# warwick-hpsc/MG-CFD-app-plain

Hardware: AMD Instinct MI355X
Metric: Medges/s (compute_flux_edge) + MG V-cycle wall-s (higher is better)
Workload: dtype f64; 1 GPU; M6-L0-like synthetic level (67^3 jittered lattice, permuted ids): 300763 nodes / 888822 internal edges per GPU, flux + update sweep, no MG; numerics=exact (bit-identical to the reference), parallelism=1 GPU, workload_kind=level0

## Files before the change

include/mgcfd.h:

```cpp
#ifndef MGCFD_H
#define MGCFD_H

#include <stdint.h>

#ifdef __cplusplus
extern "C" {
#endif

#define MGCFD_NVAR 5
#define MGCFD_RK 3

#define MGCFD_MESH_FVCORR 0
#define MGCFD_MESH_M6_WING 2
#define MGCFD_MESH_LA_CASCADE 3
#define MGCFD_MESH_ROTOR_37 4

#define MGCFD_OK 0
#define MGCFD_ERR_ARG 1
#define MGCFD_ERR_IO 2
#define MGCFD_ERR_HIP 3
#define MGCFD_ERR_NAN 4
#define MGCFD_ERR_NEG_DENSITY 5
#define MGCFD_ERR_NEG_ENERGY 6
#define MGCFD_ERR_VALIDATION 7

enum { MGCFD_LOOP_FLUX = 0, MGCFD_LOOP_UPDATE, MGCFD_LOOP_COMPUTE_STEP, MGCFD_LOOP_TIME_STEP,
       MGCFD_LOOP_RESTRICT, MGCFD_LOOP_PROLONG, MGCFD_LOOP_INDIRECT_RW, MGCFD_NUM_LOOPS };

enum { MGCFD_ARR_VARIABLES = 0, MGCFD_ARR_OLD_VARIABLES, MGCFD_ARR_FLUXES, MGCFD_ARR_RESIDUALS,
       MGCFD_ARR_STEP_FACTORS, MGCFD_ARR_VOLUMES,
       MGCFD_ARR_STAGE  };

enum {
    MGCFD_OPT_EXACT = 0,
    MGCFD_OPT_TIMING = 1,
    MGCFD_OPT_INDIRECT_RW = 2,
    MGCFD_OPT_CHECK_INVALID = 3,
    MGCFD_OPT_FLUX_VARIANT = 4,
    MGCFD_OPT_FUSE_UPDATE = 5,
    MGCFD_OPT_GRAPH = 6,
    MGCFD_OPT_RANK_SPLIT = 7,
    MGCFD_OPT_STAGE_WG4 = 8
};

typedef struct { int64_t a, b; double x, y, z; } mgcfd_edge;

typedef struct {
    int64_t nel;
    int64_t n_edges;
    int64_t n_internal, n_boundary, n_wall;
    int64_t internal_start, boundary_start, wall_start;
    const double *volumes;
    const double *coords;
    const mgcfd_edge *edges;
    const int64_t *mg_map;
    int64_t mgc;
} mgcfd_level_desc;

typedef struct mgcfd_mesh mgcfd_mesh;
typedef struct mgcfd_solver mgcfd_solver;

const char *mgcfd_last_error(void);
int mgcfd_abi_version(void);
int mgcfd_device_warm_up(int device);

int mgcfd_mesh_load(const char *input_dat, const char *directory, int duplicate, mgcfd_mesh **out);
#define MGCFD_MESH_LEGACY_ORDERING 1
int mgcfd_mesh_load_ex(const char *input_dat, const char *directory, int duplicate, int flags, mgcfd_mesh **out);
void mgcfd_mesh_free(mgcfd_mesh *m);
int mgcfd_mesh_num_levels(const mgcfd_mesh *m);
int mgcfd_mesh_variant(const mgcfd_mesh *m);
int mgcfd_mesh_size(const mgcfd_mesh *m);
int mgcfd_mesh_level(const mgcfd_mesh *m, int level, mgcfd_level_desc *out);

int mgcfd_write_array(const char *path, const double *data, int64_t nel, int ncols);
int mgcfd_identify_differences(const double *test_values, const double *master_values, int64_t nel,
                               int mesh_variant, int64_t *first_bad);

int mgcfd_create(const mgcfd_level_desc *levels, int nlevels, int mesh_variant, int device,
                 mgcfd_solver **out);
int mgcfd_create_from_mesh(const mgcfd_mesh *m, int device, mgcfd_solver **out);
int mgcfd_create_partitioned(const mgcfd_level_desc *levels, int nlevels, int mesh_variant, int device,
                             const int64_t *n_owned, mgcfd_solver **out);
int mgcfd_create_partitioned_mg(const mgcfd_level_desc *levels, int nlevels, int mesh_variant, int device,
                                const int64_t *n_owned, const int64_t *const *order_keys, mgcfd_solver **out);
int mgcfd_plan_audit(const mgcfd_level_desc *levels, int nlevels, int mesh_variant, const int64_t *n_owned,
                     const int64_t *const *order_keys, char *report, int64_t report_cap);
void mgcfd_destroy(mgcfd_solver *s);
int mgcfd_set_option(mgcfd_solver *s, int option, int value);
int mgcfd_level_has_edge_once(const mgcfd_solver *s, int level, int *yes);
int mgcfd_level_has_half_rows(const mgcfd_solver *s, int level, int *yes);
int mgcfd_level_has_order_free(const mgcfd_solver *s, int level, int *yes);
int mgcfd_level_stage_wg4(const mgcfd_solver *s, int level, int *yes);
int mgcfd_level_tiling(const mgcfd_solver *s, int level, int64_t out[10]);
int mgcfd_get_option(const mgcfd_solver *s, int option, int *value);
int mgcfd_set_stream(mgcfd_solver *s, void *hip_stream);
int mgcfd_synchronize(mgcfd_solver *s);
int mgcfd_num_levels(const mgcfd_solver *s);
int64_t mgcfd_level_nel(const mgcfd_solver *s, int level);
int64_t mgcfd_level_num_internal_edges(const mgcfd_solver *s, int level);
int mgcfd_get_far_field(const mgcfd_solver *s, double *out17);

int mgcfd_copy_old_variables(mgcfd_solver *s, int level);
int mgcfd_compute_step_factor(mgcfd_solver *s, int level);
int mgcfd_compute_flux_edge(mgcfd_solver *s, int level);
int mgcfd_compute_boundary_flux_edge(mgcfd_solver *s, int level);
int mgcfd_compute_wall_flux_edge(mgcfd_solver *s, int level);
int mgcfd_compute_fluxes(mgcfd_solver *s, int level);
int mgcfd_time_step(mgcfd_solver *s, int level, int j);
int mgcfd_zero_fluxes(mgcfd_solver *s, int level);
int mgcfd_indirect_rw(mgcfd_solver *s, int level);
int mgcfd_residual(mgcfd_solver *s, int level);
int mgcfd_calc_rms(mgcfd_solver *s, int level, double *rms);
int mgcfd_check_for_invalid_variables(mgcfd_solver *s, int level, int64_t *bad_cell);
int mgcfd_pending_invalid_state(mgcfd_solver *s, int64_t *bad_cell);
int mgcfd_restrict(mgcfd_solver *s, int fine_level);
int mgcfd_prolong(mgcfd_solver *s, int fine_level);

int mgcfd_smooth(mgcfd_solver *s, int level, int sweeps);
int mgcfd_run_cycles(mgcfd_solver *s, int cycles, double *rms_out);
int mgcfd_invalid_state_location(const mgcfd_solver *s, int64_t *cell, int *cycle);

int mgcfd_get_array(mgcfd_solver *s, int level, int which, double *out);
int mgcfd_set_array(mgcfd_solver *s, int level, int which, const double *in);
int mgcfd_array_devptr(mgcfd_solver *s, int level, int which, void **devptr, int64_t *count);
int mgcfd_array_written(mgcfd_solver *s, int level, int which);
int mgcfd_get_edges(mgcfd_solver *s, int level, mgcfd_edge *out);
int mgcfd_accept_restricted(mgcfd_solver *s, int fine_level, const void *dev_src);

int mgcfd_get_loop_iters(const mgcfd_solver *s, int level, int64_t out[MGCFD_NUM_LOOPS]);
int mgcfd_get_loop_times(mgcfd_solver *s, int level, double out_seconds[MGCFD_NUM_LOOPS]);
int mgcfd_reset_monitoring(mgcfd_solver *s);
int mgcfd_get_flux_kernel_time(mgcfd_solver *s, int level, double *avg_seconds, int64_t *launches);

int mgcfd_bench_flux(mgcfd_solver *s, int level, int launches, double *avg_seconds);
int mgcfd_bench_indirect_rw(mgcfd_solver *s, int level, int launches, double *avg_seconds);
int mgcfd_bench_stream_ceiling(mgcfd_solver *s, int level, int launches, double *avg_seconds);

int mgcfd_step_factor_local(mgcfd_solver *s, int level);
int mgcfd_step_factor_min_devptr(mgcfd_solver *s, int level, void **devptr);
int mgcfd_step_factor_apply(mgcfd_solver *s, int level);
int mgcfd_sweep_begin(mgcfd_solver *s, int level);
int mgcfd_step_factor_partials_devptr(mgcfd_solver *s, int level, void **devptr, int *count);
int mgcfd_sweep_stage(mgcfd_solver *s, int level, int j, int partials);
int mgcfd_sweep_begin_partials(mgcfd_solver *s, int level);
int mgcfd_sweep_end_partials(mgcfd_solver *s, int level);
int mgcfd_sweep_flux0(mgcfd_solver *s, int level);
int mgcfd_sweep_end(mgcfd_solver *s, int level);
int mgcfd_halo_plan(mgcfd_solver *s, int level, int64_t n, const int64_t *node_ids, int *plan);
int mgcfd_halo_pack(mgcfd_solver *s, int level, int plan, int which, void *dev_buf);
int mgcfd_halo_unpack(mgcfd_solver *s, int level, int plan, int which, const void *dev_buf);
int mgcfd_residual_sumsq(mgcfd_solver *s, int level, void **devptr);

typedef struct mgcfd_group mgcfd_group;
int mgcfd_rccl_unique_id(void *out128);
int mgcfd_rank_attach_rccl(mgcfd_solver *s, int rank, int world, const void *id128);
int mgcfd_rank_detach(mgcfd_solver *s);
int mgcfd_rank_set_halo(mgcfd_solver *s, int level, int n_peers, const int *peers, const int64_t *send_counts,
                        const int64_t *const *send_ids, const int64_t *recv_counts, const int64_t *const *recv_ids);
int mgcfd_rank_halo_info(const mgcfd_solver *s, int level, int64_t out[4]);
int mgcfd_rank_info(const mgcfd_solver *s, int out[4]);
int mgcfd_rank_graph_status(const mgcfd_solver *s, int level, int64_t out[3]);
int mgcfd_rank_exchange(mgcfd_solver *s, int level);
int mgcfd_rank_sweeps(mgcfd_solver *s, int level, int sweeps);
int mgcfd_rank_residual_sumsq(mgcfd_solver *s, int level, double *sum_all_ranks);
int mgcfd_rank_attach_plain(mgcfd_solver *s, int rank, int world);
int mgcfd_rank_ipc_export_size(mgcfd_solver *s, int level, int64_t *bytes);
int mgcfd_rank_ipc_export(mgcfd_solver *s, int level, void *out);
int mgcfd_rank_ipc_attach(mgcfd_solver *s, int level, int n_exports, const void *const *exports);
int mgcfd_rank_ipc_status(mgcfd_solver *s, int level, int *timed_out);
int mgcfd_rank_ipc_detach(mgcfd_solver *s, int level);
int mgcfd_group_create(int n, mgcfd_solver *const *solvers, mgcfd_group **out);
void mgcfd_group_destroy(mgcfd_group *g);
int mgcfd_group_exchange(mgcfd_group *g, int level);
int mgcfd_group_sweeps(mgcfd_group *g, int level, int sweeps);
int mgcfd_group_sweeps_rms(mgcfd_group *g, int level, int sweeps, double *rms_of_each);
// ... 10 lines not shown
```

mg-cfd-app-plain_amd/csrc/device_plan.hpp:

```cpp
#pragma once

#include <hip/hip_runtime.h>
#include <cstdint>

#include "preprocess.hpp"

namespace mgcfd {

constexpr int kNumStateFields = 5;
static_assert(sizeof(EdgeW) == 32, "EdgeW must be 32 bytes");
static_assert(sizeof(ProlongW) == 24, "ProlongW must be 24 bytes");

constexpr int kVariantStageWg4 = 1 << 7;

struct FarField {
    double var[5];
    double fc_mx[3], fc_my[3], fc_mz[3], fc_de[3];
};

constexpr int kMaxPushPeers = 8;
struct PushPeers {
    double *base[kMaxPushPeers] = {nullptr, nullptr, nullptr, nullptr, nullptr, nullptr, nullptr, nullptr};
    int64_t stride[kMaxPushPeers] = {0, 0, 0, 0, 0, 0, 0, 0};
    int64_t first[kMaxPushPeers + 1] = {0, 0, 0, 0, 0, 0, 0, 0, 0};
    int n = 0;
};

struct PushFlags {
    unsigned long long *flag[kMaxPushPeers] = {nullptr, nullptr, nullptr, nullptr, nullptr, nullptr, nullptr, nullptr};
    unsigned long long value = 0;
    int n = 0;
};
struct StagePush {
    const int32_t *send_ptr = nullptr;
    const int8_t *send_peer = nullptr;
    const int32_t *send_target = nullptr;
    PushPeers peers;
    PushFlags flags;
    unsigned *ticket = nullptr;
    int32_t n_boundary = 0;
};

constexpr int kMaxIpcRanks = 16;
struct FlagRows { int row[kMaxIpcRanks] = {0, 0, 0, 0, 0, 0, 0, 0, 0, 0, 0, 0, 0, 0, 0, 0}; int n = 0; };
struct MinPublish {
    double *mins[kMaxIpcRanks] = {nullptr, nullptr, nullptr, nullptr, nullptr, nullptr, nullptr, nullptr, nullptr, nullptr, nullptr, nullptr, nullptr, nullptr, nullptr, nullptr};
    unsigned long long *flag[kMaxIpcRanks] = {nullptr, nullptr, nullptr, nullptr, nullptr, nullptr, nullptr, nullptr, nullptr, nullptr, nullptr, nullptr, nullptr, nullptr, nullptr, nullptr};
    int world = 0, me = 0, parity = 0;
    unsigned long long value = 0;
};

struct FusedStep {
    double rk_div = 1.0;
    double *step_factors = nullptr;
    const double *old_variables = nullptr;
    double *q_out = nullptr;
    const double *partial_min = nullptr;
    int n_partial = 0;
    const double *volumes = nullptr;
    double *residuals = nullptr;
    const int32_t *old_of_new = nullptr;
    unsigned long long *err = nullptr;
    int check = 0;
    const double *vin_flux = nullptr;
    double vin_div = 4.0;
    int check_vin = 0;
    double *sumsq_partial = nullptr;
    double *next_partial_min = nullptr;
    const double *cbrt_vol = nullptr;
    double *next_legacy_sf = nullptr;
    const int32_t *tile_list = nullptr;
    int32_t n_list = 0;
    int64_t nel_active = 0;
};

struct SumTask {
    const double *partial = nullptr;
    int n = 0;
    double *out = nullptr;
    double *ring = nullptr;
    int *count = nullptr;
    int cap = 0;
};

struct TailPlan {
    const int32_t *rows_main = nullptr;
    const int32_t *tile_ptr = nullptr;
    const double2 *rec = nullptr;
    const int32_t *begin = nullptr, *count = nullptr;
    double2 *flux = nullptr;
};

struct DevicePlan {
    int64_t nel = 0;
    int64_t stride = 0;
    int32_t n_slices = 0;
    int32_t *slice_row0 = nullptr, *rows_int = nullptr, *rows_bnd = nullptr, *nbr = nullptr;
    double *w = nullptr;
    int32_t n_tiles = 0;
    int32_t pad_row = 0;
    int32_t pad_chunk = 0;
    uint16_t *nbr16 = nullptr;
    int32_t *tile_halo = nullptr;
    int32_t *tile_ovf_ptr = nullptr, *tile_ovf = nullptr;
    int vin_ok = 0;
    int lds_complete = 0;
    int32_t halo_max = 0;
    int edge_once = 0;
    int32_t *te_chunk_ptr = nullptr, *te_count = nullptr;
    uint16_t *te_slots = nullptr, *gat16 = nullptr;
    double *te_w = nullptr;
    double *te_w3 = nullptr;
    int half = 0;
    int free_rows = 0;
    int32_t hr_max_rows = 0;
    int free_wide = 0;
    int32_t *free_halo = nullptr;
    int32_t hr_pad_row = 0;
    int32_t *hr_row0 = nullptr;
    uint32_t *hr_code = nullptr;
    uint16_t *hg16 = nullptr;
    double *hr_w = nullptr;
    int has_tail = 0;
    TailPlan tail;
    int64_t n_edges = 0, n_edges_pad = 0;
    int32_t *fe_ab = nullptr, *row_edge = nullptr;
    double *fe_w = nullptr, *edge_flux = nullptr;
    int32_t *old_of_new = nullptr;
    int32_t *child_ptr = nullptr, *child = nullptr;
    int32_t *child4 = nullptr;
    double *pro_w = nullptr;
    int32_t *pro_p = nullptr;
    int pro_tiled = 0;
    int32_t *pro_tile_n = nullptr, *pro_tile_ids = nullptr;
    uint16_t *pro_s16 = nullptr, *pro_own16 = nullptr;
    int32_t *pro_parent = nullptr;
    double *pro_wsum = nullptr;
};

inline bool stage_wg4_fits(const DevicePlan &p) { return !p.has_tail && p.halo_max <= kTileCap4 - kTile; }

}
```

mg-cfd-app-plain_amd/csrc/kernels.hip:

```cpp
#include <hip/hip_runtime.h>
#include <algorithm>
#include <cstdlib>
#include <stdexcept>
#include <stdint.h>
#include <type_traits>

#include "device_plan.hpp"

#ifndef MGCFD_KERNEL_NS
#error "compile with -DMGCFD_KERNEL_NS=exact|fast"
#endif

namespace mgcfd {
namespace MGCFD_KERNEL_NS {

#ifdef MGCFD_PHASES
__device__ unsigned long long g_phase[4096 * 8];
__device__ unsigned long long g_phase_abs[4096 * 8];
#define PH_MARK(k) do { if (threadIdx.x == 0) { unsigned long long now_ = wall_clock64(); g_phase[(blockIdx.x & 4095) * 8 + (k)] += now_ - ph_last_; ph_last_ = now_; g_phase_abs[(blockIdx.x & 4095) * 8 + 1 + (k)] = now_; } } while (0)
#define PH_BEGIN() unsigned long long ph_last_ = wall_clock64(); if (threadIdx.x == 0) { g_phase[(blockIdx.x & 4095) * 8 + 7] += 1ull; g_phase_abs[(blockIdx.x & 4095) * 8] = ph_last_; \
        g_phase_abs[(blockIdx.x & 4095) * 8 + 7] = (static_cast<unsigned long long>(__builtin_amdgcn_s_getreg(20 | (0 << 6) | (31 << 11))) << 32) | __builtin_amdgcn_s_getreg(4 | (0 << 6) | (31 << 11)); }
#else
#define PH_MARK(k) do { } while (0)
#define PH_BEGIN() do { } while (0)
// ... 432 lines not shown
            sf_next = 0.5 * dt;
        } else if (fs.next_legacy_sf) {
            const Derived d = derive(rho, mx, my, mz, en);
            fs.next_legacy_sf[i] = 0.5 / (sqrt(fs.volumes[i]) * (d.speed + d.c));
        }
    }
    if (fs.next_partial_min || fs.sumsq_partial) {
        __shared__ double s_next[2][kBlock / 64];
        sf_next = wave_min(sf_next);
        ss = wave_sum(ss);
        if ((threadIdx.x & 63) == 0) { s_next[0][threadIdx.x >> 6] = sf_next; s_next[1][threadIdx.x >> 6] = ss; }
        __syncthreads();
        if (threadIdx.x == 0) {
            double m = s_next[0][0], sum = s_next[1][0];
            for (int wv = 1; wv < kBlock / 64; wv++) { m = fmin(m, s_next[0][wv]); sum += s_next[1][wv]; }
            if (fs.next_partial_min) fs.next_partial_min[t] = m;
            if (fs.sumsq_partial) fs.sumsq_partial[t] = sum;
        }
    }
}

__device__ __forceinline__ void boundary_rows(const NodeQ &me, const FluxC &fm, const FarField &ff,
                                              const uint16_t *__restrict__ nbr16, const double *__restrict__ w,
                                              int64_t first_row, int32_t n_bnd, int lane, int classes, double &a0,
                                              double &a1, double &a2, double &a3, double &a4)
{
    for (int32_t r = 0; r < n_bnd; r++) {
        const EdgeRow e = load_row<false>(nbr16, w, first_row + r, lane);
        const double fx = e.fx, fy = e.fy, fz = e.fz;
        if (e.code == kT16Wall && (classes & 2)) {
            a0 += 0.0;
            a1 += fx * me.p;
            a2 += fy * me.p;
            a3 += fz * me.p;
            a4 += 0.0;
        } else if (e.code == kT16Far && (classes & 4)) {
            a0 += fx * (ff.var[1] + me.mx) + fy * (ff.var[2] + me.my) + fz * (ff.var[3] + me.mz);
            a4 += fx * (ff.fc_de[0] + fm.ex) + fy * (ff.fc_de[1] + fm.ey) + fz * (ff.fc_de[2] + fm.ez);
            a1 += fx * (ff.fc_mx[0] + fm.xx) + fy * (ff.fc_mx[1] + fm.xy) + fz * (ff.fc_mx[2] + fm.xz);
            a2 += fx * (ff.fc_my[0] + fm.xy) + fy * (ff.fc_my[1] + fm.yy) + fz * (ff.fc_my[2] + fm.yz);
            a3 += fx * (ff.fc_mz[0] + fm.xz) + fy * (ff.fc_mz[1] + fm.yz) + fz * (ff.fc_mz[2] + fm.zz);
        }
    }
}

struct FluxTileLds {
    double2 tile[kTileCap * kLdsRecD2];
    double s_pm[kBlock / 64];
    double s_next[2][kBlock / 64];
};
struct FluxTileLds4 {
    double2 tile[kTileCap4 * kLdsRec80D2];
    double s_pm[kBlock / 64];
    double s_next[2][kBlock / 64];
};
static_assert(sizeof(FluxTileLds4) <= 160 * 1024 / 4, "four workgroups per CU");
static_assert(kTileCap4 - kTile < kBlock, "one halo id per thread");

template <int WMODE, bool FUSE, bool ACC, int ROLE, bool TAIL, bool PUSH, bool SLIM = false, typename Lds = FluxTileLds>
__device__ __forceinline__ void
flux_tile_body(Lds &lds, const unsigned block,
               const double *__restrict__ q, const int32_t *__restrict__ tile_halo, uint32_t n_tiles, int32_t pad_row,
               int64_t stride, int64_t nel, const int32_t *__restrict__ slice_row0,
               const int32_t *__restrict__ rows_int, const int32_t *__restrict__ rows_bnd,
               const uint16_t *__restrict__ nbr16, const double *__restrict__ w,
               const int32_t *__restrict__ tile_ovf_ptr, const int32_t *__restrict__ tile_ovf, const FarField &ff,
               double *__restrict__ fluxes, int classes, const FusedStep &fs, const TailPlan &tp,
               const uint16_t *__restrict__ gat16, const int32_t *__restrict__ te_chunk_ptr, const double *__restrict__ te_w3,
               const StagePush &push ,
               const bool block_is_tile = false )
{
    constexpr bool LOADK = WMODE == 1;
    static_assert(!PUSH || FUSE, "only a fused stage sends its message");
    PH_BEGIN();
    constexpr bool IDXW = WMODE == 2;
    static_assert(!(IDXW && TAIL), "indexed weights: levels without long rows only");
    static_assert(!SLIM || (!TAIL && !IDXW && !PUSH && ROLE != 5), "80-byte records: the stages without long rows, indexed weights, message or absorbed stage");
    double2 *const tile = lds.tile;

    double min_dt = 0.0;
    constexpr int kPartPre = 6;
    double *const s_pm = lds.s_pm;
    double pmv[kPartPre];

    const int tid = threadIdx.x;
    const int lane = tid & 63;
    unsigned t = block_is_tile ? block : xcd_contiguous_block(block, n_tiles);
    if (PUSH) {
        const unsigned nb = unsigned(push.n_boundary);
        t = block < nb ? block : nb + xcd_contiguous_block(block - nb, n_tiles - nb);
    }
    if (FUSE && fs.tile_list) t = unsigned(fs.tile_list[t]);
    const int64_t base = int64_t(t) * kTile;
    const int64_t i = base + tid;
    const int32_t slice = __builtin_amdgcn_readfirstlane(static_cast<int32_t>(i >> 6));

    const int32_t *hrow = tile_halo + int64_t(t) * kHaloStride;
    const int32_t hid = hrow[tid];
    const int32_t hid2 = (!SLIM && ROLE != 5 && tid < kHaloStride - kBlock) ? hrow[kBlock + tid] : -1;
    const int32_t row0 = slice_row0[slice];
    const int32_t n_int = (classes & 1) ? (TAIL ? tp.rows_main : rows_int)[slice] : 0;
    const int32_t n_bnd = rows_bnd[slice];
    const bool has_halo = hid >= 0;
    const int64_t hnode = has_halo ? int64_t(hid) : i;
    double o0, o1, o2, o3, o4, g0, g1, g2, g3, g4;
    EdgeRow e0, e1;
    RowRef i0{}, i1{}, i2{}, i3{};
    const double *tw = nullptr;
    if (IDXW) {
        i0 = load_ref(nbr16, gat16, n_int > 0 ? row0 : pad_row, lane);
        i1 = load_ref(nbr16, gat16, n_int > 1 ? row0 + 1 : pad_row, lane);
        i2 = load_ref(nbr16, gat16, n_int > 2 ? row0 + 2 : pad_row, lane);
        i3 = load_ref(nbr16, gat16, n_int > 3 ? row0 + 3 : pad_row, lane);
        tw = te_w3 + int64_t(te_chunk_ptr[t]) * (kEdgeChunk * 3);
    }
    if (FUSE && ROLE == 5) {
#pragma unroll
        for (int u = 0; u < kPartPre; u++) {
            const int k = threadIdx.x + u * kBlock;
            pmv[u] = fs.partial_min[k < fs.n_partial ? k : fs.n_partial - 1];
        }
        const double *od = fs.old_variables, *fl = fs.vin_flux;
        const double b0 = od[i], b1 = od[stride + i], b2 = od[2 * stride + i], b3 = od[3 * stride + i], b4 = od[4 * stride + i];
        const double f0 = fl[i], f1 = fl[stride + i], f2 = fl[2 * stride + i], f3 = fl[3 * stride + i], f4 = fl[4 * stride + i];
        const double vo = fs.volumes[i];
        const double c0 = od[hnode], c1 = od[stride + hnode], c2 = od[2 * stride + hnode], c3 = od[3 * stride + hnode],
                     c4 = od[4 * stride + hnode];
        const double h0 = fl[hnode], h1 = fl[stride + hnode], h2 = fl[2 * stride + hnode], h3 = fl[3 * stride + hnode],
                     h4 = fl[4 * stride + hnode];
        const double vh = fs.volumes[hnode];
        if (IDXW) { e0 = gather_weights(tw, i0); e1 = gather_weights(tw, i1); }
        else {
            e0 = load_row<LOADK>(nbr16, w, n_int > 0 ? row0 : pad_row, lane);
            e1 = load_row<LOADK>(nbr16, w, n_int > 1 ? row0 + 1 : pad_row, lane);
        }
        double pm = pmv[0];
#pragma unroll
        for (int u = 1; u < kPartPre; u++) pm = fmin(pm, pmv[u]);
        for (int k = threadIdx.x + kPartPre * kBlock; k < fs.n_partial; k += kBlock) pm = fmin(pm, fs.partial_min[k]);
        pm = wave_min(pm);
        if (lane == 0) s_pm[tid >> 6] = pm;
        __syncthreads();
        min_dt = s_pm[0];
        for (int wv = 1; wv < kBlock / 64; wv++) min_dt = fmin(min_dt, s_pm[wv]);
        const double fo = (min_dt / vo) / fs.vin_div, fh = (min_dt / vh) / fs.vin_div;
        o0 = b0 + fo * f0; o1 = b1 + fo * f1; o2 = b2 + fo * f2; o3 = b3 + fo * f3; o4 = b4 + fo * f4;
        g0 = c0 + fh * h0; g1 = c1 + fh * h1; g2 = c2 + fh * h2; g3 = c3 + fh * h3; g4 = c4 + fh * h4;
        if (fs.check_vin && i < nel) {
            const bool finite = isfinite(o0) && isfinite(o1) && isfinite(o2) && isfinite(o3) && isfinite(o4);
            int code = 0;
            if (!finite) code = 1;
            else if (o0 < 0.0) code = 2;
            else if (o4 < 0.0) code = 3;
            if (code) atomicMin(fs.err, err_key(fs.check_vin, fs.old_of_new[i], code));
        }
    } else {
        o0 = q[i]; o1 = q[stride + i]; o2 = q[2 * stride + i]; o3 = q[3 * stride + i]; o4 = q[4 * stride + i];
        g0 = q[hnode]; g1 = q[stride + hnode]; g2 = q[2 * stride + hnode]; g3 = q[3 * stride + hnode]; g4 = q[4 * stride + hnode];
        if (IDXW) { e0 = gather_weights(tw, i0); e1 = gather_weights(tw, i1); }
        else {
            e0 = load_row<LOADK>(nbr16, w, n_int > 0 ? row0 : pad_row, lane);
            if (!SLIM) e1 = load_row<LOADK>(nbr16, w, n_int > 1 ? row0 + 1 : pad_row, lane);
        }
    }
    if (FUSE && ROLE == 0) {
#pragma unroll
        for (int u = 0; u < kPartPre; u++) {
            const int k = threadIdx.x + u * kBlock;
            pmv[u] = fs.partial_min[k < fs.n_partial ? k : fs.n_partial - 1];
        }
    }
    const NodeQ me = make_nodeq(o0, o1, o2, o3, o4);
    lds_put_rec<SLIM>(tile, uint32_t(tid), me);
    const uint32_t hslot = (SLIM && tid >= kTileCap4 - kTile) ? uint32_t(tid) : uint32_t(kTile + tid);
    lds_put_rec<SLIM>(tile, hslot, make_nodeq(g0, g1, g2, g3, g4));
    if (hid2 >= 0) lds_store_record(tile, uint32_t(kTile + kBlock + tid), load_and_derive(q, stride, hid2));

    const FluxC fm_pre = flux_contribution(me);
    double a0 = 0.0, a1 = 0.0, a2 = 0.0, a3 = 0.0, a4 = 0.0;
    if (ACC) {
        a0 = fluxes[i]; a1 = fluxes[stride + i]; a2 = fluxes[2 * stride + i];
        a3 = fluxes[3 * stride + i]; a4 = fluxes[4 * stride + i];
    }
    const int32_t ovf0 = tile_ovf_ptr[t];
    if (FUSE && ROLE == 0) {
        double pm = pmv[0];
#pragma unroll
        for (int u = 1; u < kPartPre; u++) pm = fmin(pm, pmv[u]);
        for (int k = threadIdx.x + kPartPre * kBlock; k < fs.n_partial; k += kBlock) pm = fmin(pm, fs.partial_min[k]);
        pm = wave_min(pm);
        if (lane == 0) s_pm[tid >> 6] = pm;
    }
    PH_MARK(0);
    __syncthreads();
    PH_MARK(1);

#define MGCFD_ROW_PAIR()                                                                                     \
    do {                                                                                                     \
            const uint32_t s0 = e0.code & kT16SlotMask, s1 = e1.code & kT16SlotMask;                         \
            const bool v0 = s0 != kT16Pad, v1 = s1 != kT16Pad;                                               \
            const bool o0 = v0 && s0 >= uint32_t(kTileCap), o1 = v1 && s1 >= uint32_t(kTileCap);             \
            NodeQ n0, n1;                                                                                    \
            if (!TAIL && __builtin_expect(__any(o0 || o1), 0)) {       \
                n0 = o0 ? load_and_derive(q, stride, tile_ovf[ovf0 + int32_t(s0) - kTileCap])                \
                        : lds_load_record(tile, v0 ? s0 : uint32_t(tid));                                    \
                n1 = o1 ? load_and_derive(q, stride, tile_ovf[ovf0 + int32_t(s1) - kTileCap])                \
                        : lds_load_record(tile, v1 ? s1 : uint32_t(tid));                                    \
            } else {                                                                                         \
                n0 = lds_load_record(tile, v0 ? s0 : uint32_t(tid));                                         \
                n1 = lds_load_record(tile, v1 ? s1 : uint32_t(tid));                                         \
            }                                                                                                \
            Flux5 f0, f1;                                                                                    \
            f0 = edge_flux<LOADK>(me, fm_pre, n0, e0);                                                       \
            f1 = edge_flux<LOADK>(me, fm_pre, n1, e1);                                                       \
            if (ACC || TAIL) {                                                                               \
                a0 = v0 ? a0 + f0.d : a0;   a1 = v0 ? a1 + f0.mx : a1;   a2 = v0 ? a2 + f0.my : a2;          \
                a3 = v0 ? a3 + f0.mz : a3;  a4 = v0 ? a4 + f0.en : a4;                                       \
                a0 = v1 ? a0 + f1.d : a0;   a1 = v1 ? a1 + f1.mx : a1;   a2 = v1 ? a2 + f1.my : a2;          \
                a3 = v1 ? a3 + f1.mz : a3;  a4 = v1 ? a4 + f1.en : a4;                                       \
            } else {                                                                                         \
                a0 += f0.d; a1 += f0.mx; a2 += f0.my; a3 += f0.mz; a4 += f0.en;                              \
                a0 += f1.d; a1 += f1.mx; a2 += f1.my; a3 += f1.mz; a4 += f1.en;                              \
            }                                                                                                \
    } while (0)
    int32_t tl_b = 0, tl_e = 0, tl_nb = 0, tl_nc = 0;
    double2 tl_r0 = make_double2(0.0, 0.0), tl_r1 = tl_r0, tl_r2 = tl_r0;
    if (TAIL && (classes & 1)) {
        tl_b = tp.tile_ptr[t]; tl_e = tp.tile_ptr[t + 1];
        tl_nb = tp.begin[i]; tl_nc = tp.count[i];
        const int32_t e_first = tl_b + tid;
        if (e_first < tl_e) { tl_r0 = tp.rec[3 * int64_t(e_first)]; tl_r1 = tp.rec[3 * int64_t(e_first) + 1]; tl_r2 = tp.rec[3 * int64_t(e_first) + 2]; }
    }
    double r0 = 0.0, r1 = 0.0, r2 = 0.0, r3 = 0.0, r4 = 0.0, sfv = 0.0;
#define MGCFD_ROW_ONE()                                                                                      \
    do {                                                                                                     \
            const uint32_t s0 = e0.code & kT16SlotMask;                                                      \
            const bool v0 = s0 != kT16Pad;                                                                   \
            const NodeQ n0 = lds_get_record80(tile, v0 ? s0 : uint32_t(tid));                              \
            const Flux5 f0 = edge_flux<LOADK>(me, fm_pre, n0, e0);                                           \
            if (ACC) {                                                                                       \
                a0 = v0 ? a0 + f0.d : a0;   a1 = v0 ? a1 + f0.mx : a1;   a2 = v0 ? a2 + f0.my : a2;          \
                a3 = v0 ? a3 + f0.mz : a3;  a4 = v0 ? a4 + f0.en : a4;                                       \
            } else {                                                                                         \
                a0 += f0.d; a1 += f0.mx; a2 += f0.my; a3 += f0.mz; a4 += f0.en;                              \
            }                                                                                                \
    } while (0)
    if (SLIM) {
        int32_t r = 0;
        for (; r + 1 < n_int; r++) {
            const EdgeRow e1n = load_row<LOADK>(nbr16, w, row0 + r + 1, lane);
            MGCFD_ROW_ONE();
            e0 = e1n;
        }
        if (FUSE) {
            if (ROLE == 0) {
                r0 = me.rho; r1 = me.mx; r2 = me.my; r3 = me.mz; r4 = me.en;
            } else {
                r0 = fs.old_variables[i]; r1 = fs.old_variables[stride + i]; r2 = fs.old_variables[2 * stride + i];
                r3 = fs.old_variables[3 * stride + i]; r4 = fs.old_variables[4 * stride + i];
            }
            sfv = (ROLE == 0 ? fs.volumes : fs.step_factors)[i];
        }
        if (r < n_int) MGCFD_ROW_ONE();
    } else
    {
        int32_t r = 0;
        if (IDXW) {
            for (; r + 2 < n_int; r += 2) {
                const RowRef i4 = load_ref(nbr16, gat16, r + 4 < n_int ? row0 + r + 4 : pad_row, lane);
                const RowRef i5 = load_ref(nbr16, gat16, r + 5 < n_int ? row0 + r + 5 : pad_row, lane);
                const EdgeRow e2 = gather_weights(tw, i2), e3 = gather_weights(tw, i3);
                MGCFD_ROW_PAIR();
                e0 = e2; e1 = e3; i2 = i4; i3 = i5;
            }
        } else
        for (; r + 2 < n_int; r += 2) {
            const EdgeRow e2 = load_row<LOADK>(nbr16, w, row0 + r + 2, lane);
            const EdgeRow e3 = load_row<LOADK>(nbr16, w, r + 3 < n_int ? row0 + r + 3 : pad_row, lane);
            MGCFD_ROW_PAIR();
            e0 = e2; e1 = e3;
        }
        if (FUSE) {
            if (ROLE == 0) {
                r0 = me.rho; r1 = me.mx; r2 = me.my; r3 = me.mz; r4 = me.en;
            } else {
                r0 = fs.old_variables[i]; r1 = fs.old_variables[stride + i]; r2 = fs.old_variables[2 * stride + i];
                r3 = fs.old_variables[3 * stride + i]; r4 = fs.old_variables[4 * stride + i];
            }
            sfv = ((ROLE == 0 || ROLE == 5) ? fs.volumes : fs.step_factors)[i];
        }
        if (r < n_int) MGCFD_ROW_PAIR();
    }
#undef MGCFD_ROW_PAIR
#undef MGCFD_ROW_ONE
    PH_MARK(2);

    if (TAIL && (classes & 1) && tl_e > tl_b) {
        const int32_t last0 = tl_b + ((tl_e - tl_b - 1) / kBlock) * kBlock;
        int32_t e = tl_b + tid;
        double2 r0 = tl_r0, r1 = tl_r1, r2 = tl_r2;
        Flux5 fl;
        fl.d = 0.0; fl.mx = 0.0; fl.my = 0.0; fl.mz = 0.0; fl.en = 0.0;
        while (e < tl_e) {
            const double2 c0 = r0, c1 = r1, c2 = r2;
            const int32_t en = e + kBlock;
            if (en < tl_e) { r0 = tp.rec[3 * int64_t(en)]; r1 = tp.rec[3 * int64_t(en) + 1]; r2 = tp.rec[3 * int64_t(en) + 2]; }
            const uint32_t word = static_cast<uint32_t>(__double_as_longlong(c2.x));
            const uint32_t own = word & 0xFFFFu;
            if (own != kT16Pad) {
                EdgeRow er;
                er.code = word >> 16;
                er.fx = c0.x; er.fy = c0.y; er.fz = c1.x; er.k = LOADK ? c1.y : 0.0;
                const uint32_t s = er.code & kT16SlotMask;
                const NodeQ mo = lds_load_record(tile, own);
                const NodeQ ot = s >= uint32_t(kTileCap) ? load_and_derive(q, stride, tile_ovf[ovf0 + int32_t(s) - kTileCap])
                                                         : lds_load_record(tile, s);
                const Flux5 f = edge_flux<LOADK>(mo, flux_contribution(mo), ot, er);
                if (e >= last0) {
                    fl = f;
                } else {
                    double2 *out = tp.flux + 3 * int64_t(e);
                    out[0] = make_double2(f.d, f.mx); out[1] = make_double2(f.my, f.mz); out[2] = make_double2(f.en, 0.0);
                }
            }
            e = en;
        }
        asm volatile("s_waitcnt vmcnt(0)" ::: "memory");
        __syncthreads();
        tile[3 * tid] = make_double2(fl.d, fl.mx); tile[3 * tid + 1] = make_double2(fl.my, fl.mz); tile[3 * tid + 2] = make_double2(fl.en, 0.0);
        __syncthreads();
        const int32_t n_glob = min(tl_nc, max(0, last0 - tl_nb));
#define MGCFD_ADD_ENTRIES(in, count)                                                                              \
        do {                                                                                                      \
            int32_t k_ = 0;                                                                                       \
            for (; k_ + 3 <= (count); k_ += 3) {            \
                const double2 u0 = in[0], u1 = in[1], u2 = in[2], v0 = in[3], v1 = in[4], v2 = in[5],              \
                              w0 = in[6], w1 = in[7], w2 = in[8];                                                 \
                in += 9;                                                                                          \
                a0 += u0.x; a1 += u0.y; a2 += u1.x; a3 += u1.y; a4 += u2.x;                                       \
                a0 += v0.x; a1 += v0.y; a2 += v1.x; a3 += v1.y; a4 += v2.x;                                       \
                a0 += w0.x; a1 += w0.y; a2 += w1.x; a3 += w1.y; a4 += w2.x;                                       \
            }                                                                                                     \
            for (; k_ < (count); k_++) {                                                                          \
                const double2 u0 = in[0], u1 = in[1], u2 = in[2];                                                 \
                in += 3;                                                                                          \
                a0 += u0.x; a1 += u0.y; a2 += u1.x; a3 += u1.y; a4 += u2.x;                                       \
            }                                                                                                     \
        } while (0)
        if (n_glob > 0) {
            const double2 *in = tp.flux + 3 * int64_t(tl_nb);
            MGCFD_ADD_ENTRIES(in, n_glob);
        }
        {
            const double2 *in = tile + 3 * (tl_nb + n_glob - last0);
            const int32_t n_lds = tl_nc - n_glob;
            MGCFD_ADD_ENTRIES(in, n_lds);
        }
#undef MGCFD_ADD_ENTRIES
    }

    if ((classes & 6) && n_bnd > 0) {
        const int32_t first_bnd = rows_int[slice];
        const FluxC fm = fm_pre;
        for (int32_t r = 0; r < n_bnd; r++) {
            const EdgeRow e = load_row<false>(nbr16, w, int64_t(row0) + first_bnd + r, lane);
            const double fx = e.fx, fy = e.fy, fz = e.fz;
            if (e.code == kT16Wall && (classes & 2)) {
                a0 += 0.0;
                a1 += fx * me.p;
                a2 += fy * me.p;
                a3 += fz * me.p;
                a4 += 0.0;
            } else if (e.code == kT16Far && (classes & 4)) {
                a0 += fx * (ff.var[1] + me.mx) + fy * (ff.var[2] + me.my) + fz * (ff.var[3] + me.mz);
                a4 += fx * (ff.fc_de[0] + fm.ex) + fy * (ff.fc_de[1] + fm.ey) + fz * (ff.fc_de[2] + fm.ez);
                a1 += fx * (ff.fc_mx[0] + fm.xx) + fy * (ff.fc_mx[1] + fm.xy) + fz * (ff.fc_mx[2] + fm.xz);
                a2 += fx * (ff.fc_my[0] + fm.xy) + fy * (ff.fc_my[1] + fm.yy) + fz * (ff.fc_my[2] + fm.yz);
                a3 += fx * (ff.fc_mz[0] + fm.xz) + fy * (ff.fc_mz[1] + fm.yz) + fz * (ff.fc_mz[2] + fm.zz);
            }
        }
    }

    if (!FUSE) {
        if (i < nel) {
            MGCFD_ST_FLUX(fluxes + i, a0); MGCFD_ST_FLUX(fluxes + stride + i, a1); MGCFD_ST_FLUX(fluxes + 2 * stride + i, a2);
            MGCFD_ST_FLUX(fluxes + 3 * stride + i, a3); MGCFD_ST_FLUX(fluxes + 4 * stride + i, a4);
        }
        PH_MARK(3);
        return;
    }
    double sf_next = __longlong_as_double(0x7FF0000000000000LL);
    double ss = 0.0;
    if (i < nel) {
        double sf = sfv;
        if (ROLE == 0 || ROLE == 5) {
            min_dt = s_pm[0];
            for (int wv = 1; wv < kBlock / 64; wv++) min_dt = fmin(min_dt, s_pm[wv]);
            sf = min_dt / sfv;
            fs.step_factors[i] = sf;
        }
        const double factor = sf / fs.rk_div;
        const double rho = r0 + factor * a0, mx = r1 + factor * a1, my = r2 + factor * a2, mz = r3 + factor * a3,
                     en = r4 + factor * a4;
        store_conserved(fs.q_out, stride, i, rho, mx, my, mz, en);
        if (ROLE >= 2 && ROLE <= 4) {
            const double d0 = rho - r0, d1 = mx - r1, d2 = my - r2, d3 = mz - r3, d4 = en - r4;
            if (fs.residuals) {
                MGCFD_ST_STAGE(fs.residuals + i, d0); MGCFD_ST_STAGE(fs.residuals + stride + i, d1); MGCFD_ST_STAGE(fs.residuals + 2 * stride + i, d2);
                MGCFD_ST_STAGE(fs.residuals + 3 * stride + i, d3); MGCFD_ST_STAGE(fs.residuals + 4 * stride + i, d4);
            }
            if (fs.sumsq_partial) ss = (((d0 * d0 + d1 * d1) + d2 * d2) + d3 * d3) + d4 * d4;
        }
        if (fs.check) {
            const bool finite = isfinite(rho) && isfinite(mx) && isfinite(my) && isfinite(mz) && isfinite(en);
            int code = 0;
            if (!finite) code = 1;
            else if (rho < 0.0) code = 2;
            else if (en < 0.0) code = 3;
            if (code) atomicMin(fs.err, err_key(fs.check, fs.old_of_new[i], code));
        }
        if (ROLE == 3) {
            const Derived d = derive(rho, mx, my, mz, en);
            const double dt = fs.cbrt_vol[i] / (d.speed + d.c);
            sf_next = 0.5 * dt;
        } else if (ROLE == 4) {
            const Derived d = derive(rho, mx, my, mz, en);
            fs.next_legacy_sf[i] = 0.5 / (sqrt(fs.volumes[i]) * (d.speed + d.c));
        }
        if (PUSH && block < unsigned(push.n_boundary)) {
            for (int32_t e = push.send_ptr[i]; e < push.send_ptr[i + 1]; e++) {
                const int k = push.send_peer[e];
                const int64_t g = push.send_target[e];
                double *dst = push.peers.base[0];
                int64_t ps = push.peers.stride[0];
#pragma unroll
                for (int p = 1; p < kMaxPushPeers; p++) if (p == k) { dst = push.peers.base[p]; ps = push.peers.stride[p]; }
                dst[g] = rho; dst[ps + g] = mx; dst[2 * ps + g] = my; dst[3 * ps + g] = mz; dst[4 * ps + g] = en;
            }
        }
    }
    if (PUSH && block < unsigned(push.n_boundary)) {
        asm volatile("s_waitcnt vmcnt(0)" ::: "memory");
        __syncthreads();
        if (threadIdx.x == 0) {
            __threadfence_system();
            const unsigned done = __hip_atomic_fetch_add(push.ticket, 1u, __ATOMIC_ACQ_REL, __HIP_MEMORY_SCOPE_AGENT);
            if (done == unsigned(push.n_boundary) - 1u) {
                __hip_atomic_store(push.ticket, 0u, __ATOMIC_RELAXED, __HIP_MEMORY_SCOPE_AGENT);
                __threadfence_system();
#pragma unroll
                for (int p = 0; p < kMaxPushPeers; p++)
                    if (p < push.flags.n) __hip_atomic_store(push.flags.flag[p], push.flags.value, __ATOMIC_RELEASE, __HIP_MEMORY_SCOPE_SYSTEM);
            }
        }
    }
    if (ROLE == 3 || (ROLE >= 2 && ROLE <= 4 && fs.sumsq_partial)) {
        double (*const s_next)[kBlock / 64] = lds.s_next;
        if (ROLE == 3) sf_next = wave_min(sf_next);
        if (fs.sumsq_partial) ss = wave_sum(ss);
        if ((threadIdx.x & 63) == 0) { s_next[0][threadIdx.x >> 6] = sf_next; s_next[1][threadIdx.x >> 6] = ss; }
        __syncthreads();
        if (threadIdx.x == 0) {
            double m = s_next[0][0], sum = s_next[1][0];
            for (int wv = 1; wv < kBlock / 64; wv++) { m = fmin(m, s_next[0][wv]); sum += s_next[1][wv]; }
            if (ROLE == 3) fs.next_partial_min[t] = m;
            if (fs.sumsq_partial) fs.sumsq_partial[t] = sum;
        }
    }
    PH_MARK(3);
}

template <int MINW, int WMODE, bool FUSE, bool ACC, int ROLE, bool TAIL, bool PUSH = false, bool SLIM = false>
__global__ void __launch_bounds__(kBlock, MINW)
k_flux_tile(
            const double *__restrict__ q, const int32_t *__restrict__ tile_halo, uint32_t n_tiles, int32_t pad_row,
            int64_t stride, int64_t nel, const int32_t *__restrict__ slice_row0,
            const int32_t *__restrict__ rows_int, const int32_t *__restrict__ rows_bnd,
            const uint16_t *__restrict__ nbr16, const double *__restrict__ w,
            const int32_t *__restrict__ tile_ovf_ptr, const int32_t *__restrict__ tile_ovf, FarField ff,
            double *__restrict__ fluxes, int classes, FusedStep fs, TailPlan tp,
            const uint16_t *__restrict__ gat16, const int32_t *__restrict__ te_chunk_ptr, const double *__restrict__ te_w3,
            StagePush push)
{
    __shared__ std::conditional_t<SLIM, FluxTileLds4, FluxTileLds> lds;
    flux_tile_body<WMODE, FUSE, ACC, ROLE, TAIL, PUSH, SLIM>(lds, blockIdx.x, q, tile_halo, n_tiles, pad_row, stride, nel, slice_row0, rows_int, rows_bnd, nbr16, w,
                                                       tile_ovf_ptr, tile_ovf, ff, fluxes, classes, fs, tp, gat16, te_chunk_ptr, te_w3, push);
}

struct TileEdge { uint32_t sa, sb; double fx, fy, fz, k; };
constexpr int kGatherPre = 8;

template <bool LOADK>
__device__ __forceinline__ TileEdge load_tile_edge(const uint16_t *__restrict__ te_slots, const double *__restrict__ te_w,
                                                   int64_t chunk, int tid)
{
    TileEdge e;
    e.sa = te_slots[(chunk * 2) * kEdgeChunk + tid];
    e.sb = te_slots[(chunk * 2 + 1) * kEdgeChunk + tid];
    const double *wr = te_w + chunk * (4 * kEdgeChunk) + tid;
    e.fx = wr[0]; e.fy = wr[kEdgeChunk]; e.fz = wr[2 * kEdgeChunk];
    e.k = LOADK ? wr[3 * kEdgeChunk] : 0.0;
    return e;
}

__device__ __forceinline__ TileEdge no_tile_edge()
{
    TileEdge e;
    e.sa = kT16Pad; e.sb = kT16Pad; e.fx = 0.0; e.fy = 0.0; e.fz = 0.0; e.k = 0.0;
    return e;
}

template <bool LOADK, bool FUSE, bool ACC>
__global__ void __launch_bounds__(kBlock, 3)
k_flux_edge_once(const double *__restrict__ q, const int32_t *__restrict__ tile_halo, uint32_t n_tiles, int32_t pad_row,
                 int64_t stride, int64_t nel, const int32_t *__restrict__ te_chunk_ptr,
                 const int32_t *__restrict__ te_count, int32_t pad_chunk, int classes,
                 const int32_t *__restrict__ slice_row0,
                 const int32_t *__restrict__ rows_int, const int32_t *__restrict__ rows_bnd,
                 const uint16_t *__restrict__ nbr16, const double *__restrict__ w, const uint16_t *__restrict__ gat16,
                 const uint16_t *__restrict__ te_slots, const double *__restrict__ te_w,
                 const int32_t *__restrict__ tile_ovf_ptr, const int32_t *__restrict__ tile_ovf, FarField ff,
                 double *__restrict__ fluxes, FusedStep fs)
{
    __shared__ double2 tile[kTileCap * kLdsRecD2];

    double min_dt = 0.0;
    if (FUSE && fs.partial_min) min_dt = block_min_of_partials(fs.partial_min, fs.n_partial);

    const unsigned t = xcd_contiguous_block(blockIdx.x, n_tiles);
    const int tid = threadIdx.x;
    const int lane = tid & 63;
    const int wave_base = tid & ~63;
    const int64_t base = int64_t(t) * kTile;
    const int64_t i = base + tid;
    const int32_t slice = __builtin_amdgcn_readfirstlane(static_cast<int32_t>(i >> 6));

    const int32_t *hrow = tile_halo + int64_t(t) * kHaloStride;
    const int32_t hid = hrow[tid];
    const int32_t hid2 = tid < kHaloStride - kBlock ? hrow[kBlock + tid] : -1;
    const double o0 = q[i], o1 = q[stride + i], o2 = q[2 * stride + i], o3 = q[3 * stride + i], o4 = q[4 * stride + i];
    const int32_t n_te = te_count[t];
    const int64_t chunk0 = te_chunk_ptr[t];
    TileEdge e_cur = load_tile_edge<LOADK>(te_slots, te_w, wave_base < n_te ? chunk0 : pad_chunk, tid);
    TileEdge e_nxt = load_tile_edge<LOADK>(te_slots, te_w, kEdgeChunk + wave_base < n_te ? chunk0 + 1 : pad_chunk, tid);

    const int32_t row0 = slice_row0[slice];
    const int32_t n_int = rows_int[slice];
    const int32_t n_bnd = rows_bnd[slice];
// ... 1154 lines not shown
            double *d = cr + k * 5;
            d[0] = coarse_residuals[c2]; d[1] = coarse_residuals[sc + c2]; d[2] = coarse_residuals[2 * sc + c2];
            d[3] = coarse_residuals[3 * sc + c2]; d[4] = coarse_residuals[4 * sc + c2];
        }
    }
    __syncthreads();

    const double *od = cr + own_slot * 5;
    const double o0 = od[0], o1 = od[1], o2 = od[2], o3 = od[3], o4 = od[4];
    double r0, r1, r2, r3, r4;
    if (parent < 0) {
        r0 = o0; r1 = o1; r2 = o2; r3 = o3; r4 = o4;
    } else {
        r0 = r1 = r2 = r3 = r4 = 0.0;
#define MGCFD_PRO_PAIR(R)                                                                                      \
        do {                                                                                                   \
            const bool v0 = wa0 != 0.0 || wb0 != 0.0;                                                          \
            const bool v1 = ((R) + 1 < n_int) && (wa1 != 0.0 || wb1 != 0.0);                                   \
            const double *xd0 = cr + (v0 ? sl0 : own_slot) * 5, *xd1 = cr + (v1 ? sl1 : own_slot) * 5;         \
            const double x00 = xd0[0], x01 = xd0[1], x02 = xd0[2], x03 = xd0[3], x04 = xd0[4];                 \
            const double x10 = xd1[0], x11 = xd1[1], x12 = xd1[2], x13 = xd1[3], x14 = xd1[4];                 \
            if (v0) {                                                                                          \
                r0 += wa0 * o0; r1 += wa0 * o1; r2 += wa0 * o2; r3 += wa0 * o3; r4 += wa0 * o4;                \
                r0 += wb0 * x00; r1 += wb0 * x01; r2 += wb0 * x02; r3 += wb0 * x03; r4 += wb0 * x04;           \
            }                                                                                                  \
            if (v1) {                                                                                          \
                r0 += wa1 * o0; r1 += wa1 * o1; r2 += wa1 * o2; r3 += wa1 * o3; r4 += wa1 * o4;                \
                r0 += wb1 * x10; r1 += wb1 * x11; r2 += wb1 * x12; r3 += wb1 * x13; r4 += wb1 * x14;           \
            }                                                                                                  \
        } while (0)
        int32_t r = 0;
        for (; r + 2 < n_int; r += 2, wr += 256, sr += 128) {
            const double wa2 = wr[256], wb2 = wr[320], wa3 = wr[384], wb3 = wr[448];
            const uint32_t sl2 = sr[128], sl3 = sr[192];
            MGCFD_PRO_PAIR(r);
            wa0 = wa2; wb0 = wb2; wa1 = wa3; wb1 = wb3; sl0 = sl2; sl1 = sl3;
        }
        if (r < n_int) MGCFD_PRO_PAIR(r);
#undef MGCFD_PRO_PAIR
    }
    double sf = __longlong_as_double(0x7FF0000000000000LL);
    if (active) {
        const double n0 = q0 + (f0 - r0 / ws);
        const double n1 = q1 + (f1 - r1 / ws);
        const double n2 = q2 + (f2 - r2 / ws);
        const double n3 = q3 + (f3 - r3 / ws);
        const double n4 = q4 + (f4 - r4 / ws);
        store_conserved(fine_q, stride, i, n0, n1, n2, n3, n4);
        if (partial_min) sf = local_step_factor(n0, n1, n2, n3, n4, cbrt_vol[i]);
    }
    if (partial_min) block_min_to(sf, partial_min);
}

static inline unsigned grid_for(int64_t n) { return static_cast<unsigned>((n + kBlock - 1) / kBlock); }

void launch_init_variables(hipStream_t st, int64_t stride, const FarField &ff, double *q)
{ hipLaunchKernelGGL(k_init_variables, dim3(grid_for(stride)), dim3(kBlock), 0, st, stride, ff, q); }

void launch_step_factor_local(hipStream_t st, int64_t nel, int64_t stride, const double *q, const double *cbrt_vol,
                              double *sf, double *partial_min, double *old_variables)
{ hipLaunchKernelGGL(k_step_factor_local, dim3(grid_for(nel)), dim3(kBlock), 0, st, nel, stride, q, cbrt_vol, sf, partial_min, old_variables); }

void launch_min_reduce(hipStream_t st, int64_t nel, const double *partial_min, double *out)
{ hipLaunchKernelGGL(k_min_reduce, dim3(1), dim3(kBlock), 0, st, partial_min, int(grid_for(nel)), out); }

void launch_step_factor_apply(hipStream_t st, int64_t nel, const double *min_dt_scalar,
                              const double *volumes, double *sf)
{ hipLaunchKernelGGL(k_step_factor_apply, dim3(grid_for(nel)), dim3(kBlock), 0, st, nel, min_dt_scalar, volumes, sf); }

void launch_step_factor_legacy(hipStream_t st, int64_t nel, int64_t stride, const double *q, const double *volumes, double *sf,
                               double *old_variables)
{ hipLaunchKernelGGL(k_step_factor_legacy, dim3(grid_for(nel)), dim3(kBlock), 0, st, nel, stride, q, volumes, sf, old_variables); }

void launch_flux(hipStream_t st, const DevicePlan &p, const double *q, const FarField &ff, double *fluxes,
                 int classes, int accumulate, int variant, const FusedStep *fused, const StagePush *push)
{
    const dim3 block(kBlock);
    FusedStep fs{};
    if (fused) fs = *fused;
    const bool part = fused && fs.tile_list;
    const int64_t nel_arg = (fused && fs.nel_active > 0) ? fs.nel_active : p.nel;
    const dim3 grid(part ? fs.n_list : p.n_tiles);
    if (part && fs.n_list <= 0) return;

#define MGCFD_TILE_LAUNCH_T(WMODE, FUSE, ACC, ROLE, TAIL)                                                      \
    hipLaunchKernelGGL((k_flux_tile<((TAIL) && ((ACC) || (ROLE) == 5)) ? 2 : 3, WMODE, FUSE, ACC, ROLE, TAIL>), grid, block, 0, st, q, p.tile_halo,     \
                       uint32_t(grid.x), p.pad_row, p.stride, nel_arg, p.slice_row0, p.rows_int, p.rows_bnd, \
                       p.nbr16, p.w, p.tile_ovf_ptr, p.tile_ovf, ff, fluxes, classes, fs, p.tail, p.gat16,     \
                       p.te_chunk_ptr, p.te_w3, StagePush{})
    const bool tail = p.has_tail && (classes & 1);
    if (push && fused && part && !fs.vin_flux) {
        const int role_p = fs.partial_min ? 0 : (fs.next_partial_min ? 3 : (fs.next_legacy_sf ? 4 : (fs.residuals ? 2 : 1)));
#define MGCFD_PUSH_LAUNCH_T(WMODE, ROLE, TAIL)                                                                  \
    hipLaunchKernelGGL((k_flux_tile<3, WMODE, true, false, ROLE, TAIL, true>), grid, block, 0, st, q, p.tile_halo,     \
                       uint32_t(grid.x), p.pad_row, p.stride, nel_arg, p.slice_row0, p.rows_int, p.rows_bnd, \
                       p.nbr16, p.w, p.tile_ovf_ptr, p.tile_ovf, ff, fluxes, classes, fs, p.tail, p.gat16,     \
                       p.te_chunk_ptr, p.te_w3, *push)
#define MGCFD_PUSH_LAUNCH_R(WMODE, TAIL)                                                                        \
    do {                                                                                                       \
        if (role_p == 0) MGCFD_PUSH_LAUNCH_T(WMODE, 0, TAIL);                                                  \
        else if (role_p == 2) MGCFD_PUSH_LAUNCH_T(WMODE, 2, TAIL);                                             \
        else if (role_p == 3) MGCFD_PUSH_LAUNCH_T(WMODE, 3, TAIL);                                             \
        else if (role_p == 4) MGCFD_PUSH_LAUNCH_T(WMODE, 4, TAIL);                                             \
        else MGCFD_PUSH_LAUNCH_T(WMODE, 1, TAIL);                                                              \
    } while (0)
        if (role_p == 0 && q != fs.old_variables) throw std::logic_error("a first stage whose input is not the sweep's start state");
        const bool k_streamed = (variant & 1) == 0;
        if (tail) { if (k_streamed) MGCFD_PUSH_LAUNCH_R(1, true); else MGCFD_PUSH_LAUNCH_R(0, true); }
        else { if (k_streamed) MGCFD_PUSH_LAUNCH_R(1, false); else MGCFD_PUSH_LAUNCH_R(0, false); }
#undef MGCFD_PUSH_LAUNCH_R
#undef MGCFD_PUSH_LAUNCH_T
        return;
    }
    const bool indexed = (variant & 16) && p.edge_once && p.te_w3 && !tail;
#define MGCFD_TILE_LAUNCH_R(LOADK, FUSE, ACC, ROLE)                                                            \
    do {                                                                                                       \
        if (tail) MGCFD_TILE_LAUNCH_T(LOADK ? 1 : 0, FUSE, ACC, ROLE, true);                                   \
        else if (indexed) MGCFD_TILE_LAUNCH_T(2, FUSE, ACC, ROLE, false);                                      \
        else MGCFD_TILE_LAUNCH_T(LOADK ? 1 : 0, FUSE, ACC, ROLE, false);                                       \
    } while (0)
    const int role = !fused ? 1 : (fs.vin_flux ? 5 : fs.partial_min ? 0 : (fs.next_partial_min ? 3 : (fs.next_legacy_sf ? 4 : (fs.residuals ? 2 : 1))));
    if (role == 0 && q != fs.old_variables) throw std::logic_error("a first stage whose input is not the sweep's start state");
#define MGCFD_TILE_LAUNCH(LOADK, FUSE, ACC)                                                                    \
    do {                                                                                                       \
        if (role == 0) MGCFD_TILE_LAUNCH_R(LOADK, FUSE, ACC, 0);                                               \
        else if (role == 2) MGCFD_TILE_LAUNCH_R(LOADK, FUSE, ACC, 2);                                          \
        else if (role == 3) MGCFD_TILE_LAUNCH_R(LOADK, FUSE, ACC, 3);                                          \
        else if (role == 4) MGCFD_TILE_LAUNCH_R(LOADK, FUSE, ACC, 4);                                          \
        else if (role == 5) MGCFD_TILE_LAUNCH_R(LOADK, FUSE, ACC, 5);                                          \
        else MGCFD_TILE_LAUNCH_R(LOADK, FUSE, ACC, 1);                                                         \
    } while (0)
    if ((variant & 4) && !fused && p.edge_flux) {
        if (classes & 1)
            hipLaunchKernelGGL(k_fission_edge_flux, dim3(grid_for(p.n_edges)), block, 0, st, p.n_edges, p.n_edges_pad, p.stride, q,
                               p.fe_ab, p.fe_w, p.edge_flux);
        if (accumulate)
            hipLaunchKernelGGL(k_fission_node_sum<true>, grid, block, 0, st, p.nel, p.stride, p.n_edges_pad, q, p.slice_row0,
                               p.rows_int, p.rows_bnd, p.row_edge, p.nbr16, p.w, p.edge_flux, ff, fluxes, classes);
        else
            hipLaunchKernelGGL(k_fission_node_sum<false>, grid, block, 0, st, p.nel, p.stride, p.n_edges_pad, q, p.slice_row0,
                               p.rows_int, p.rows_bnd, p.row_edge, p.nbr16, p.w, p.edge_flux, ff, fluxes, classes);
        return;
    }
#ifdef MGCFD_ORDER_FREE
    if ((variant & 64) && p.free_rows && (classes & 1) && !(fused && fs.vin_flux) && !part && !(fused && fs.nel_active > 0)) {
#define MGCFD_FREE_LAUNCH_L(FUSE, ACC, CAP, LONG)                                                               \
    hipLaunchKernelGGL((k_flux_free<FUSE, ACC, CAP, LONG>), grid, block, 0, st, q, p.tile_halo, uint32_t(p.n_tiles), \
                       p.hr_pad_row, p.stride, p.nel, p.hr_row0, p.hr_code, p.hr_w, p.slice_row0,               \
                       p.rows_int, p.rows_bnd, p.nbr16, p.w, ff, fluxes, classes, fs)
#define MGCFD_FREE_LAUNCH_C(FUSE, ACC, CAP)                                                                     \
    do { if (p.hr_max_rows > kHalfMaxRows) MGCFD_FREE_LAUNCH_L(FUSE, ACC, CAP, true); else MGCFD_FREE_LAUNCH_L(FUSE, ACC, CAP, false); } while (0)
#define MGCFD_FREE_LAUNCH_W(FUSE, ACC)                                                                          \
    hipLaunchKernelGGL((k_flux_free<FUSE, ACC, kTile + kFreeHaloStride, true, true>), grid, block, 0, st, q, p.free_halo, uint32_t(p.n_tiles), \
                       p.hr_pad_row, p.stride, p.nel, p.hr_row0, p.hr_code, p.hr_w, p.slice_row0,               \
                       p.rows_int, p.rows_bnd, p.nbr16, p.w, ff, fluxes, classes, fs)
        static const bool wg3 = std::getenv("MGCFD_FREE_WG3") && std::atoi(std::getenv("MGCFD_FREE_WG3")) != 0;
#define MGCFD_FREE_LAUNCH(FUSE, ACC)                                                                            \
    do { if (p.free_wide) MGCFD_FREE_LAUNCH_W(FUSE, ACC);                                                       \
         else if (p.halo_max <= kFreeCap4 - kTile && !wg3) MGCFD_FREE_LAUNCH_C(FUSE, ACC, kFreeCap4); else MGCFD_FREE_LAUNCH_C(FUSE, ACC, kTileCap); } while (0)
        const int role_f = !fused ? -1 : (fs.next_legacy_sf ? -1 : (fs.partial_min ? 0 : (fs.next_partial_min ? 3 : ((fs.residuals || fs.sumsq_partial) ? 2 : 1))));
        static const bool no_roles = std::getenv("MGCFD_FREE_NO_ROLES") && std::atoi(std::getenv("MGCFD_FREE_NO_ROLES")) != 0;
        const bool fast_path = !p.free_wide && p.halo_max <= kFreeCap4 - kTile && !wg3 && p.hr_max_rows <= kHalfMaxRows;
#define MGCFD_FREE_LAUNCH_ROLE(ROLE)                                                                            \
    hipLaunchKernelGGL((k_flux_free<true, false, kFreeCap4, false, false, ROLE>), grid, block, 0, st, q, p.tile_halo, uint32_t(p.n_tiles), \
                       p.hr_pad_row, p.stride, p.nel, p.hr_row0, p.hr_code, p.hr_w, p.slice_row0,               \
                       p.rows_int, p.rows_bnd, p.nbr16, p.w, ff, fluxes, classes, fs)
        if (fused && role_f >= 0 && fast_path && !no_roles && !(role_f == 0 && q != fs.old_variables)) {
            if (role_f == 0) MGCFD_FREE_LAUNCH_ROLE(0);
            else if (role_f == 2) MGCFD_FREE_LAUNCH_ROLE(2);
            else if (role_f == 3) MGCFD_FREE_LAUNCH_ROLE(3);
            else MGCFD_FREE_LAUNCH_ROLE(1);
        }
        else if (fused) MGCFD_FREE_LAUNCH(true, false);
        else if (accumulate) MGCFD_FREE_LAUNCH(false, true);
        else MGCFD_FREE_LAUNCH(false, false);
#undef MGCFD_FREE_LAUNCH_ROLE
#undef MGCFD_FREE_LAUNCH_C
#undef MGCFD_FREE_LAUNCH_L
#undef MGCFD_FREE_LAUNCH_W
#undef MGCFD_FREE_LAUNCH
        return;
    }
#endif
    if ((variant & 32) && p.half && (classes & 1) && !(fused && fs.vin_flux) && !part) {
#define MGCFD_HALF_LAUNCH(FUSE, ACC)                                                                            \
    hipLaunchKernelGGL((k_flux_half<FUSE, ACC>), grid, block, 0, st, q, p.tile_halo, uint32_t(p.n_tiles),       \
                       p.hr_pad_row, p.stride, p.nel, p.hr_row0, p.hr_code, p.hr_w, p.hg16, p.slice_row0,       \
                       p.rows_int, p.rows_bnd, p.pad_row, p.nbr16, p.w, ff, fluxes, classes, fs)
        if (fused) MGCFD_HALF_LAUNCH(true, false);
        else if (accumulate) MGCFD_HALF_LAUNCH(false, true);
        else MGCFD_HALF_LAUNCH(false, false);
#undef MGCFD_HALF_LAUNCH
        return;
    }
    const bool loadk = (variant & 1) == 0;
    if ((variant & 2) && p.edge_once && (classes & 1) && !part) {
#define MGCFD_EO_LAUNCH(LOADK, FUSE, ACC)                                                                      \
    hipLaunchKernelGGL((k_flux_edge_once<LOADK, FUSE, ACC>), grid, block, 0, st, q, p.tile_halo,               \
                       uint32_t(p.n_tiles), p.pad_row, p.stride, p.nel, p.te_chunk_ptr, p.te_count,            \
                       p.pad_chunk, classes, p.slice_row0, p.rows_int, p.rows_bnd, p.nbr16, p.w, p.gat16,      \
                       p.te_slots, p.te_w, p.tile_ovf_ptr, p.tile_ovf, ff, fluxes, fs)
        if (fused) {
            if (loadk) MGCFD_EO_LAUNCH(true, true, false); else MGCFD_EO_LAUNCH(false, true, false);
        } else if (accumulate) {
            if (loadk) MGCFD_EO_LAUNCH(true, false, true); else MGCFD_EO_LAUNCH(false, false, true);
        } else {
            if (loadk) MGCFD_EO_LAUNCH(true, false, false); else MGCFD_EO_LAUNCH(false, false, false);
        }
#undef MGCFD_EO_LAUNCH
        return;
    }
#ifndef MGCFD_ORDER_FREE
    if (fused && (variant & kVariantStageWg4) && stage_wg4_fits(p) && !indexed && role != 5) {
#define MGCFD_SLIM_LAUNCH_T(WMODE, ROLE)                                                                        \
    hipLaunchKernelGGL((k_flux_tile<4, WMODE, true, false, ROLE, false, false, true>), grid, block, 0, st, q, p.tile_halo, \
                       uint32_t(grid.x), p.pad_row, p.stride, nel_arg, p.slice_row0, p.rows_int, p.rows_bnd, \
                       p.nbr16, p.w, p.tile_ovf_ptr, p.tile_ovf, ff, fluxes, classes, fs, p.tail, p.gat16,     \
                       p.te_chunk_ptr, p.te_w3, StagePush{})
#define MGCFD_SLIM_LAUNCH_R(WMODE)                                                                              \
    do {                                                                                                       \
        if (role == 0) MGCFD_SLIM_LAUNCH_T(WMODE, 0);                                                          \
        else if (role == 2) MGCFD_SLIM_LAUNCH_T(WMODE, 2);                                                     \
        else if (role == 3) MGCFD_SLIM_LAUNCH_T(WMODE, 3);                                                     \
        else if (role == 4) MGCFD_SLIM_LAUNCH_T(WMODE, 4);                                                     \
        else MGCFD_SLIM_LAUNCH_T(WMODE, 1);                                                                    \
    } while (0)
        if (loadk) MGCFD_SLIM_LAUNCH_R(1); else MGCFD_SLIM_LAUNCH_R(0);
#undef MGCFD_SLIM_LAUNCH_R
#undef MGCFD_SLIM_LAUNCH_T
        return;
    }
#endif
    if (fused) {
        if (loadk) MGCFD_TILE_LAUNCH(true, true, false); else MGCFD_TILE_LAUNCH(false, true, false);
    } else if (accumulate) {
        if (loadk) MGCFD_TILE_LAUNCH(true, false, true); else MGCFD_TILE_LAUNCH(false, false, true);
    } else {
        if (loadk) MGCFD_TILE_LAUNCH(true, false, false); else MGCFD_TILE_LAUNCH(false, false, false);
    }
#undef MGCFD_TILE_LAUNCH
#undef MGCFD_TILE_LAUNCH_R
#undef MGCFD_TILE_LAUNCH_T
}

__global__ void __launch_bounds__(kBlock)
k_stream_tiles(const double2 *__restrict__ src, double *__restrict__ dst, int64_t rd_total2, int64_t wr_total, int rd2_per_thread, int wr_per_thread)
{
    __shared__ double lds[40960 / 8 - 64];
    const int64_t r0 = int64_t(blockIdx.x) * rd2_per_thread * kBlock + threadIdx.x;
    double acc = 0.0;
    for (int k = 0; k < rd2_per_thread; k += 8) {
        double2 v[8];
#pragma unroll
        for (int u = 0; u < 8; u++) {
            const int64_t j = r0 + int64_t(k + u) * kBlock;
            v[u] = src[(k + u < rd2_per_thread && j < rd_total2) ? j : int64_t(threadIdx.x)];
        }
#pragma unroll
        for (int u = 0; u < 8; u++) acc += v[u].x + v[u].y;
    }
    if (acc == 1.2345e300) { lds[threadIdx.x] = acc; __syncthreads(); acc = lds[(threadIdx.x + 1) & 255]; }
    const int64_t w0 = int64_t(blockIdx.x) * wr_per_thread * kBlock + threadIdx.x;
    for (int k = 0; k < wr_per_thread; k++) {
        const int64_t j = w0 + int64_t(k) * kBlock;
        if (j < wr_total) MGCFD_ST_FLUX(dst + j, acc + double(k));
    }
}

void launch_stream_tiles(hipStream_t st, int n_tiles, const double *src, double *dst, int64_t rd_total, int64_t wr_total)
{
    const int64_t rd2 = rd_total / 2;
    const int rd2_per_thread = int((rd2 + int64_t(n_tiles) * kBlock - 1) / (int64_t(n_tiles) * kBlock));
    const int wr_per_thread = int((wr_total + int64_t(n_tiles) * kBlock - 1) / (int64_t(n_tiles) * kBlock));
    hipLaunchKernelGGL(k_stream_tiles, dim3(n_tiles), dim3(kBlock), 0, st, reinterpret_cast<const double2 *>(src), dst, rd2, wr_total, rd2_per_thread, wr_per_thread);
}

void launch_indirect_rw(hipStream_t st, const DevicePlan &p, const double *q, double *fluxes, int variant)
{
    if (p.lds_complete && !p.has_tail && !(variant & 8)) {
// ... 108 lines not shown
```

mg-cfd-app-plain_amd/csrc/solver.cpp:

```cpp
#include <hip/hip_runtime.h>
#include <dlfcn.h>

#include <functional>
#include <future>

#include <algorithm>
#include <atomic>
#include <cmath>
#include <cstdio>
#include <cstdlib>
#include <chrono>
#include <cstring>
#include <limits>
#include <map>
#include <memory>
#include <mutex>
#include <stdexcept>
#include <string>
#include <thread>
#include <vector>

#include "kernels.hpp"
#include "mesh.hpp"
#include "mgcfd.h"
// ... 17 lines not shown
template <typename T> static T *dev_alloc(size_t n)
{
    void *p = nullptr;
    HIP_CHECK(hipMalloc(&p, (n ? n : 1) * sizeof(T)));
    return static_cast<T *>(p);
}

template <typename T> static T *dev_upload(const std::vector<T> &v)
{
    T *p = dev_alloc<T>(v.size());
    if (!v.empty()) HIP_CHECK(hipMemcpy(p, v.data(), v.size() * sizeof(T), hipMemcpyHostToDevice));
    return p;
}

struct LevelStaging {
    struct Item { std::function<void(char *)> place; const void *src; size_t bytes; size_t offset; };
    std::vector<Item> items;
    std::vector<std::shared_ptr<void>> keep;
    size_t total = 0;
    static constexpr size_t kAlign = 4096;
    template <typename F> void alloc(F *&field, size_t bytes, const void *src = nullptr)
    {
        const size_t off = total;
        total += (std::max<size_t>(bytes, 1) + kAlign - 1) / kAlign * kAlign;
        F **where = &field;
        items.push_back({[where, off](char *base) { *where = reinterpret_cast<F *>(base + off); }, src, src ? bytes : 0, off});
    }
    template <typename F, typename T> void upload(F *&field, const std::vector<T> &v) { alloc(field, v.size() * sizeof(T), v.data()); }
    template <typename F, typename T> void upload(F *&field, std::vector<T> &&v)
    {
        auto held = std::make_shared<std::vector<T>>(std::move(v));
        keep.push_back(held);
        upload(field, *held);
    }
};

struct EventPair { hipEvent_t start, stop; int level, loop; bool is_flux_internal; int launches; };

struct HaloExchange {
    static constexpr int kSets = 3;
    std::vector<int> peer;
    std::vector<int64_t> send_off, recv_off;
    int32_t *send_idx = nullptr, *recv_idx = nullptr;
    double *send_buf[kSets] = {nullptr, nullptr, nullptr}, *recv_buf[kSets] = {nullptr, nullptr, nullptr};
    int32_t *tiles_boundary = nullptr, *tiles_interior = nullptr, *tiles_all = nullptr;
    int32_t n_boundary = 0, n_interior = 0;
    hipStream_t comm_stream = nullptr;
    hipEvent_t packed[kSets] = {nullptr, nullptr, nullptr}, arrived[kSets] = {nullptr, nullptr, nullptr};
    hipEvent_t reduced = nullptr, gathered = nullptr, joined = nullptr;
    double *gmin = nullptr;
    double *min_par = nullptr;
    int min_parity = 0;
    const double **peer_scalars[2] = {nullptr, nullptr};
    hipGraphExec_t sweep_graph[6] = {nullptr, nullptr, nullptr, nullptr, nullptr, nullptr};
    int64_t graph_iters[6][MGCFD_NUM_LOOPS] = {{0}};
    bool graph_failed = false;
    int64_t sweeps_replayed = 0;
    std::vector<int32_t> recv_idx_host;
    int32_t *push_target = nullptr;
    hipEvent_t bdone[3] = {nullptr, nullptr, nullptr};
    bool direct = false;
    bool ipc = false;
    unsigned long long *flags = nullptr;
    double *gmins = nullptr;
    bool ipc_all = false;
    unsigned long long sweep_seq = 0;
    double *all_mins[kMaxIpcRanks] = {};
    unsigned long long *all_flag[kMaxIpcRanks] = {};
    unsigned *ticket = nullptr;
    int *ipc_timeouts = nullptr;
    bool ipc_unacknowledged = false;
    unsigned long long seq = 0;
    double *peer_state[kMaxPushPeers][3] = {};
    int64_t peer_stride[kMaxPushPeers] = {};
    int peer_rot_delta[kMaxPushPeers] = {};
    unsigned long long *peer_flag[kMaxPushPeers] = {};
    std::vector<void *> ipc_opened;
    int32_t *node_send_ptr = nullptr, *node_send_target = nullptr;
    int8_t *node_send_peer = nullptr;
    int64_t total_send() const { return send_off.empty() ? 0 : send_off.back(); }
    int64_t total_recv() const { return recv_off.empty() ? 0 : recv_off.back(); }
};

struct DeviceLevel {
    mgcfd_level_desc info{};
    std::vector<mgcfd_edge> edges;
    LevelPlan plan;
    DevicePlan dp;
    double *q = nullptr, *old_variables = nullptr, *fluxes = nullptr, *residuals = nullptr;
    double *q_alt = nullptr;
    double *state[3] = {nullptr, nullptr, nullptr};
    int rot = 0;
    void apply_rot() { q = state[rot % 3]; q_alt = state[(rot + 1) % 3]; old_variables = state[(rot + 2) % 3]; }
    double *tile_sumsq = nullptr;
    bool want_sumsq = false;
    bool have_sumsq = false;
    int64_t row_bytes = 0;
    bool min_ahead = false;
    double *sf_alt = nullptr;
    int sf_par = 0;
    double *sfb[2] = {nullptr, nullptr};
    void apply_sf() { step_factors = sfb[sf_par & 1]; sf_alt = sfb[(sf_par & 1) ^ 1]; }
    double *step_factors = nullptr, *volumes = nullptr, *cbrt_vol = nullptr;
    double *min_dt = nullptr;
    double *partial_min = nullptr;
    double *sumsq = nullptr, *partials = nullptr;
    int n_partials = 0;
    bool fluxes_zero = true;
    bool fluxes_stale = false;
    bool residuals_stale = false;
    bool sweep_flux0_done = false;
    int stage_next = 0;
    double *stage_out = nullptr;
    int64_t n_owned = 0;
    std::vector<std::pair<int32_t *, int64_t>> halo_plans;
    std::unique_ptr<HaloExchange> hx;
    bool has_transfer = false;
    void *block = nullptr;
    size_t block_bytes = 0;
    bool in_block(const void *p) const { return block && p >= block && p < static_cast<const char *>(block) + block_bytes; }
    int64_t iters[MGCFD_NUM_LOOPS] = {0};
    double times[MGCFD_NUM_LOOPS] = {0};
    double flux_time = 0.0;
    int64_t flux_launches = 0;
    int64_t att_sweeps = 0, att_sweeps_sampled = 0;
    int64_t att_calls[MGCFD_NUM_LOOPS] = {0}, att_calls_sampled[MGCFD_NUM_LOOPS] = {0};
};

}

using namespace mgcfd;

struct mgcfd_mesh { HostMesh mesh; };

struct mgcfd_solver {
    int device = 0;
    int mesh_variant = 0;
    hipStream_t own_stream = nullptr, stream = nullptr;
    std::vector<DeviceLevel> L;
    FarField ff{};
    double ff17[17] = {0};
    unsigned long long *err = nullptr;
    int opt_exact = 1, opt_timing = 0, opt_indirect_rw = 0, opt_check = 1, opt_variant = -1, opt_fuse = 1, opt_graph = 0, opt_stage_wg4 = 1;
    int opt_rank_split = 1;
    bool opt_lazy_residual = !(std::getenv("MGCFD_LAZY_RESIDUAL") && std::atoi(std::getenv("MGCFD_LAZY_RESIDUAL")) == 0);
    int check_seq = 0;
    int64_t invalid_cell = -1; int invalid_cycle = -1;
    int next_check() { if (!opt_check) return 0; if (check_seq < (1 << 22)) check_seq++; return check_seq; }
    int force_check = -1;
    int timing_stride = 8;
    double att_total = 0.0;
    bool probe_first_stage_only = false;
    int64_t sweep_counter = 0;
    bool in_timed_group = false;
    struct SweepGraph { hipGraphExec_t exec = nullptr; int64_t iters[MGCFD_NUM_LOOPS] = {0}; bool ahead_after = false; int rot_after = 0; int sf_par_after = 0; bool sumsq_after = false, res_stale_after = false; };
    std::map<uint64_t, SweepGraph> sweep_graphs;
    struct CycleGraph { hipGraphExec_t exec = nullptr; std::vector<std::vector<int64_t>> iters; std::vector<bool> ahead_after, res_stale_after; std::vector<int> rot_after, sf_par_after; };
    std::map<uint64_t, CycleGraph> cycle_graphs;
    static constexpr int kRmsRing = 4096;
    double *rms_ring = nullptr;
    int *rms_count = nullptr;
    std::vector<EventPair> pending;
    std::vector<hipEvent_t> free_events;

    ~mgcfd_solver();
    void use_device() const { HIP_CHECK(hipSetDevice(device)); }
    DeviceLevel &level(int l)
    {
        if (l < 0 || l >= static_cast<int>(L.size())) throw std::invalid_argument("level out of range");
        return L[static_cast<size_t>(l)];
    }

    hipEvent_t get_event()
    {
        if (pending.size() >= 8192) fold_events();
        if (!free_events.empty()) { hipEvent_t e = free_events.back(); free_events.pop_back(); return e; }
        hipEvent_t e;
        HIP_CHECK(hipEventCreate(&e));
        return e;
    }
    void fold_events()
    {
        if (pending.empty()) return;
        HIP_CHECK(hipStreamSynchronize(stream));
        for (auto &p : pending) {
            float ms = 0.f;
            HIP_CHECK(hipEventElapsedTime(&ms, p.start, p.stop));
            DeviceLevel &lv = L[static_cast<size_t>(p.level)];
            lv.times[p.loop] += double(ms) * 1e-3;
            if (p.is_flux_internal) { lv.flux_time += double(ms) * 1e-3; lv.flux_launches += p.launches; }
            free_events.push_back(p.start);
            free_events.push_back(p.stop);
        }
        pending.clear();
    }
    struct Timed {
        mgcfd_solver *s; EventPair p; bool on;
        Timed(mgcfd_solver *s_, int level, int loop, bool flux_internal = false, int launches = 1)
            : s(s_), on(!s_->in_timed_group && (s_->opt_timing == 1 || (s_->opt_timing == 2 && flux_internal)))
        {
            if (!on) return;
            p = EventPair{s->get_event(), s->get_event(), level, loop, flux_internal, launches};
            if (launches > 1) s->in_timed_group = true;
            HIP_CHECK(hipEventRecord(p.start, s->stream));
        }
        ~Timed()
        {
            if (!on) return;
            (void)hipEventRecord(p.stop, s->stream);
            s->pending.push_back(p);
            if (p.launches > 1) s->in_timed_group = false;
        }
    };

    void op_copy_old(int l)
    {
        DeviceLevel &lv = level(l);
        settle_residuals(lv);
        HIP_CHECK(hipMemcpyAsync(lv.old_variables, lv.q, sizeof(double) * 5 * lv.dp.stride, hipMemcpyDeviceToDevice, stream));
    }
    void op_step_factor_local(int l, bool fuse_copy_old, bool reduce_to_scalar)
    {
        DeviceLevel &lv = level(l);
        lv.min_ahead = false;
        if (fuse_copy_old) settle_residuals(lv);
        double *old = fuse_copy_old ? lv.old_variables : nullptr;
        if (opt_exact) exact::launch_step_factor_local(stream, lv.info.nel, lv.dp.stride, lv.q, lv.cbrt_vol, lv.step_factors, lv.partial_min, old);
        else fast::launch_step_factor_local(stream, lv.info.nel, lv.dp.stride, lv.q, lv.cbrt_vol, lv.step_factors, lv.partial_min, old);
        if (reduce_to_scalar) exact::launch_min_reduce(stream, lv.info.nel, lv.partial_min, lv.min_dt);
    }
    void op_step_factor_apply(int l)
    {
        DeviceLevel &lv = level(l);
        if (opt_exact) exact::launch_step_factor_apply(stream, lv.info.nel, lv.min_dt, lv.volumes, lv.step_factors);
        else fast::launch_step_factor_apply(stream, lv.info.nel, lv.min_dt, lv.volumes, lv.step_factors);
    }
    void settle_residuals(DeviceLevel &lv)
    {
        if (!lv.residuals_stale) return;
        lv.residuals_stale = false;
        if (opt_exact) exact::launch_residual(stream, lv.dp.stride, lv.old_variables, lv.q, lv.residuals);
        else fast::launch_residual(stream, lv.dp.stride, lv.old_variables, lv.q, lv.residuals);
    }
    void settle_fluxes(DeviceLevel &lv)
    {
        if (!lv.fluxes_stale) return;
        HIP_CHECK(hipMemsetAsync(lv.fluxes, 0, sizeof(double) * 5 * lv.dp.stride, stream));
        lv.fluxes_stale = false;
    }
    bool op_step_factor(int l, bool fused = false, bool copy_old = true)
    {
        DeviceLevel &lv = level(l);
        Timed t(this, l, MGCFD_LOOP_COMPUTE_STEP);
        bool apply_pending = false;
        if (mesh_variant == MGCFD_MESH_FVCORR) {
            double *old = (fused && copy_old) ? lv.old_variables : nullptr;
            if (old) settle_residuals(lv);
            if (opt_exact) exact::launch_step_factor_legacy(stream, lv.info.nel, lv.dp.stride, lv.q, lv.volumes, lv.step_factors, old);
            else fast::launch_step_factor_legacy(stream, lv.info.nel, lv.dp.stride, lv.q, lv.volumes, lv.step_factors, old);
        } else {
            op_step_factor_local(l, fused && copy_old, !fused);
            if (fused) apply_pending = true;
            else op_step_factor_apply(l);
        }
        lv.iters[MGCFD_LOOP_COMPUTE_STEP] += lv.info.nel;
        return apply_pending;
    }
    void upload_optional_plans(DeviceLevel &lv)
    {
        LevelPlan &P = lv.plan;
        const int v = opt_variant;
        auto take = [](auto &vec) { auto *p = dev_upload(vec); vec.clear(); vec.shrink_to_fit(); return p; };
        if (lv.dp.free_rows && !lv.dp.hr_code && (!opt_exact || (v >= 0 && (v & (32 | 64))))) {
            lv.dp.hr_row0 = dev_upload(P.hr_row0);
            lv.dp.hr_code = take(P.hr_code);
            lv.dp.hr_w = take(P.hr_w);
            if (lv.dp.free_wide) lv.dp.free_halo = take(P.free_halo);
        }
        if (lv.dp.free_rows && !lv.dp.hg16 && v >= 0 && (v & 32)) lv.dp.hg16 = take(P.hg16);
        if (lv.dp.edge_once && !lv.dp.gat16 && v >= 0 && (v & (2 | 16))) {
            lv.dp.te_chunk_ptr = dev_upload(P.te_chunk_ptr);
            lv.dp.te_count = dev_upload(P.te_count);
            lv.dp.gat16 = take(P.gat16);
            {
                const size_t n_chunks = P.te_w.size() / (4 * kEdgeChunk);
                std::vector<double> w3(n_chunks * kEdgeChunk * 3);
                for (size_t c = 0; c < n_chunks; c++)
                    for (size_t ln = 0; ln < size_t(kEdgeChunk); ln++)
                        for (size_t k = 0; k < 3; k++) w3[(c * kEdgeChunk + ln) * 3 + k] = P.te_w[(c * 4 + k) * kEdgeChunk + ln];
                lv.dp.te_w3 = dev_upload(w3);
            }
            lv.dp.te_slots = take(P.te_slots);
            lv.dp.te_w = take(P.te_w);
        }
        if (!lv.dp.fe_ab && v >= 0 && (v & 4)) {
            lv.dp.fe_ab = take(P.fe_ab);
            lv.dp.fe_w = take(P.fe_w);
            lv.dp.row_edge = take(P.row_edge);
        }
        if (!lv.dp.nbr && ((v >= 0 && (v & 8)) || !lv.dp.lds_complete || lv.dp.has_tail)) lv.dp.nbr = take(P.nbr);
    }
    void upload_optional_plans()
    {
        use_device();
        for (DeviceLevel &lv : L) upload_optional_plans(lv);
    }
    int variant_for(const DeviceLevel &lv, bool fused = false) const
    {
        if (opt_variant >= 0) return opt_variant;
        const bool free_fast_path = !lv.dp.free_wide && lv.dp.halo_max <= kFreeCap4Halo && lv.dp.hr_max_rows <= kHalfMaxRows;
        if (!opt_exact && lv.dp.free_rows && (!fused || lv.dp.free_wide || lv.dp.has_tail || free_fast_path)) return 1 | 64;
        return 1;
    }
    mutable int n_cus = 0;
    bool stage_wg4_for(const DeviceLevel &lv) const
    {
        if (!opt_exact || !opt_stage_wg4 || !stage_wg4_fits(lv.dp)) return false;
        if (n_cus == 0) {
            use_device();
            HIP_CHECK(hipDeviceGetAttribute(&n_cus, hipDeviceAttributeMultiprocessorCount, device));
        }
        return lv.dp.n_tiles > 3 * n_cus;
    }
    void op_flux(int l, int classes)
    {
        DeviceLevel &lv = level(l);
        Timed t(this, l, MGCFD_LOOP_FLUX, (classes & 1) != 0);
        if (classes != 7) settle_fluxes(lv);
        const int accumulate = lv.fluxes_zero ? 0 : 1;
        const int variant = variant_for(lv);
        if ((variant & 4) && !lv.dp.edge_flux)
            lv.dp.edge_flux = dev_alloc<double>(static_cast<size_t>(lv.dp.n_edges_pad) * 5 + 8);
        if (opt_exact) exact::launch_flux(stream, lv.dp, lv.q, ff, lv.fluxes, classes, accumulate, variant, nullptr);
        else fast::launch_flux(stream, lv.dp, lv.q, ff, lv.fluxes, classes, accumulate, variant, nullptr);
        lv.fluxes_zero = false;
        lv.fluxes_stale = false;
        if (classes & 1) lv.iters[MGCFD_LOOP_FLUX] += lv.info.n_internal;
    }
    void op_fused_stage(int l, int j, const double *in, double *out, int apply_min, bool with_residual,
                        const double *old = nullptr, bool look_ahead = false, bool sumsq = false,
                        const double *vin_flux = nullptr, const int32_t *tile_list = nullptr, int32_t n_list = 0,
                        bool count_iters = true, const double *min_list = nullptr, int n_min = 0, bool lazy_residual = false,
                        const StagePush *push = nullptr)
    {
        DeviceLevel &lv = level(l);
        const FusedStep fs = fused_step(l, j, out, apply_min, with_residual, old, look_ahead, sumsq, vin_flux, tile_list, n_list, min_list, n_min, lazy_residual);
        Timed t(this, l, MGCFD_LOOP_FLUX, true);
        if (opt_exact) exact::launch_flux(stream, lv.dp, in, ff, lv.fluxes, 7, 0, variant_for(lv, true) | (stage_wg4_for(lv) ? kVariantStageWg4 : 0), &fs, push);
        else fast::launch_flux(stream, lv.dp, in, ff, lv.fluxes, 7, 0, variant_for(lv, true), &fs, push);
        if (count_iters) {
            lv.iters[MGCFD_LOOP_FLUX] += lv.info.n_internal;
            lv.iters[MGCFD_LOOP_TIME_STEP] += lv.info.nel;
        }
    }
    FusedStep fused_step(int l, int j, double *out, int apply_min, bool with_residual, const double *old, bool look_ahead, bool sumsq,
                         const double *vin_flux, const int32_t *tile_list, int32_t n_list, const double *min_list, int n_min, bool lazy_residual)
    {
        DeviceLevel &lv = level(l);
        settle_residuals(lv);
        FusedStep fs;
        fs.tile_list = tile_list;
        fs.n_list = n_list;
        if (tile_list && lv.plan.ghosts_last && lv.n_owned < lv.info.nel) fs.nel_active = lv.n_owned;
        fs.rk_div = double(MGCFD_RK + 1 - j);
        fs.step_factors = lv.step_factors;
        fs.old_variables = old ? old : lv.old_variables;
        fs.q_out = out;
        fs.next_partial_min = (look_ahead && mesh_variant != MGCFD_MESH_FVCORR) ? lv.partial_min : nullptr;
        fs.next_legacy_sf = (look_ahead && mesh_variant == MGCFD_MESH_FVCORR) ? lv.sf_alt : nullptr;
        fs.cbrt_vol = lv.cbrt_vol;
        if (out == lv.q) lv.min_ahead = false;
        fs.partial_min = apply_min == 1 ? lv.partial_min : (apply_min == 2 ? lv.min_dt : (apply_min == 3 ? min_list : nullptr));
        fs.n_partial = apply_min == 2 ? 1 : (apply_min == 3 ? n_min : static_cast<int>((lv.info.nel + 255) / 256));
        fs.volumes = lv.volumes;
        fs.residuals = (with_residual && !lazy_residual) ? lv.residuals : nullptr;
        fs.sumsq_partial = (with_residual && sumsq) ? lv.tile_sumsq : nullptr;
        fs.vin_flux = vin_flux;
        fs.vin_div = double(MGCFD_RK + 1);
        fs.old_of_new = lv.dp.old_of_new;
        fs.err = err;
        if (vin_flux) fs.check_vin = next_check();
        fs.check = force_check >= 0 ? force_check : next_check();
        return fs;
    }
    void op_indirect_rw(int l)
    {
        DeviceLevel &lv = level(l);
        settle_fluxes(lv);
        Timed t(this, l, MGCFD_LOOP_INDIRECT_RW);
        if (opt_exact) exact::launch_indirect_rw(stream, lv.dp, lv.q, lv.fluxes, variant_for(lv));
        else fast::launch_indirect_rw(stream, lv.dp, lv.q, lv.fluxes, variant_for(lv));
        lv.fluxes_zero = false;
        lv.iters[MGCFD_LOOP_INDIRECT_RW] += lv.info.n_internal;
    }
    void op_zero_fluxes(int l)
    {
        DeviceLevel &lv = level(l);
        HIP_CHECK(hipMemsetAsync(lv.fluxes, 0, sizeof(double) * 5 * lv.dp.stride, stream));
        lv.fluxes_zero = true;
        lv.fluxes_stale = false;
    }
    void op_time_step(int l, int j, int apply_min = 0, bool with_residual = false, bool lazy_zero = false,
                      const double *old = nullptr, double *out = nullptr)
    {
        if (j < 0 || j >= MGCFD_RK) throw std::invalid_argument("RK stage out of range");
        DeviceLevel &lv = level(l);
        settle_fluxes(lv);
        settle_residuals(lv);
        if (!old) old = lv.old_variables;
        if (!out) out = lv.q;
        if (out == lv.q) lv.min_ahead = false;
        Timed t(this, l, MGCFD_LOOP_TIME_STEP);
        const double *pm = apply_min == 1 ? lv.partial_min : (apply_min == 2 ? lv.min_dt : nullptr);
        const int n_pm = apply_min == 2 ? 1 : static_cast<int>((lv.info.nel + 255) / 256);
        double *res = with_residual ? lv.residuals : nullptr;
        const int check = next_check();
        if (opt_exact) exact::launch_time_step(stream, lv.info.nel, lv.dp.stride, j, lv.step_factors, lv.fluxes, old, out, lv.dp.old_of_new, err, check, pm, n_pm, lv.volumes, res, lazy_zero ? 0 : 1);
        else fast::launch_time_step(stream, lv.info.nel, lv.dp.stride, j, lv.step_factors, lv.fluxes, old, out, lv.dp.old_of_new, err, check, pm, n_pm, lv.volumes, res, lazy_zero ? 0 : 1);
        lv.fluxes_stale = lazy_zero;
        lv.fluxes_zero = true;
        lv.iters[MGCFD_LOOP_TIME_STEP] += lv.info.nel;
    }
    void op_residual(int l)
    {
        DeviceLevel &lv = level(l);
        lv.residuals_stale = false;
        if (opt_exact) exact::launch_residual(stream, lv.dp.stride, lv.old_variables, lv.q, lv.residuals);
        else fast::launch_residual(stream, lv.dp.stride, lv.old_variables, lv.q, lv.residuals);
    }
// ... 180 lines not shown
        PlanOptions &popt = popt_l;
        const mgcfd_level_desc &d = levels[l];
        DeviceLevel &lv = s->L[static_cast<size_t>(l)];
        if (!d.volumes || !d.edges) throw std::invalid_argument("level is missing volumes/edges");
        if (d.internal_start < 0 || d.internal_start + d.n_internal > d.n_edges || d.boundary_start < 0 ||
            d.boundary_start + d.n_boundary > d.n_edges || d.wall_start < 0 || d.wall_start + d.n_wall > d.n_edges)
            throw std::invalid_argument("edge class ranges exceed n_edges");
        lv.edges.assign(d.edges, d.edges + d.n_edges);
        adjust_and_dampen(d, mesh_variant, lv.edges);
        lv.n_owned = d.nel;
        popt.n_owned = -1;
        if (n_owned && n_owned[l] >= 0 && n_owned[l] < d.nel) {
            lv.n_owned = n_owned[l];
            popt.n_owned = n_owned[l];
        }
        popt.long_rows = !std::getenv("MGCFD_NO_LONG_ROWS");
        build_level_plan(d, lv.edges, popt, lv.plan);
        if (std::getenv("MGCFD_VERBOSE"))
            std::fprintf(stderr, "[mgcfd] level %d: %ld nodes, %d tiles, halo mean %.0f max %d (cap %d), overflow refs %ld, ELL padding %.1f%%, tile edges mean %.0f max %d (edge-once %s)\n",
                         l, (long)d.nel, lv.plan.n_tiles, lv.plan.halo_mean, lv.plan.halo_max, kTileCap - kTile,
                         (long)lv.plan.halo_overflow_refs, 100.0 * lv.plan.pad_fraction, lv.plan.te_mean, lv.plan.te_max,
                         lv.plan.edge_once ? "yes" : "no");
        if (std::getenv("MGCFD_VERBOSE"))
            std::fprintf(stderr, "[mgcfd] level %d: half rows %s: %ld evaluations (%.2f per node), %ld in another node's lane, %ld padding slots (%.1f%%)\n", l, lv.plan.half ? "yes" : "no",
                         (long)lv.plan.hr_entries, double(lv.plan.hr_entries) / double(d.nel), (long)lv.plan.hr_foreign, (long)lv.plan.hr_padding,
                         lv.plan.hr_entries ? 100.0 * double(lv.plan.hr_padding) / double(lv.plan.hr_entries) : 0.0);
        if (std::getenv("MGCFD_VERBOSE")) {
            const int64_t nt = lv.plan.n_tiles, q8 = nt >> 3, r8 = nt & 7;
            auto xcd_of = [&](int64_t t) { return t < r8 * (q8 + 1) ? t / (q8 + 1) : r8 + (t - r8 * (q8 + 1)) / std::max<int64_t>(q8, 1); };
            int64_t total = 0, foreign = 0, near_ = 0;
            for (int64_t t = 0; t < nt; t++)
                for (int32_t k = lv.plan.tile_halo_ptr[static_cast<size_t>(t)]; k < lv.plan.tile_halo_ptr[static_cast<size_t>(t) + 1]; k++) {
                    const int64_t o = lv.plan.tile_halo[static_cast<size_t>(k)] / kTile;
                    total++;
                    if (xcd_of(o) != xcd_of(t)) foreign++;
                    else if (std::llabs(o - t) <= 48) near_++;
                }
            std::fprintf(stderr, "[mgcfd] level %d: staged halo nodes %ld: %.1f%% owned by a tile of another XCD's range, %.1f%% by a tile within 48 of the reader in its own range\n",
                         l, (long)total, total ? 100.0 * foreign / total : 0.0, total ? 100.0 * near_ / total : 0.0);
        }
        if (std::getenv("MGCFD_VERBOSE") && lv.plan.has_tail) {
            int64_t rows_full = 0, rows_cut = 0;
            for (size_t q = 0; q < lv.plan.rows_int.size(); q++) { rows_full += lv.plan.rows_int[q]; rows_cut += lv.plan.rows_main[q]; }
            std::fprintf(stderr, "[mgcfd] level %d: long rows: %ld entries left to the workgroups (%.1f per tile), per-node loop %.1f -> %.1f rows per slice\n",
                         l, (long)lv.plan.tail_total, double(lv.plan.tail_total) / lv.plan.n_tiles,
                         double(rows_full) / double(lv.plan.rows_int.size()), double(rows_cut) / double(lv.plan.rows_int.size()));
        }
    });
    lap("level plans (a thread per level)");
    run_per_level(nlevels - 1, [&](int l) {
        const mgcfd_level_desc &d = levels[l];
        if (!d.mg_map) throw std::invalid_argument("multigrid map missing between levels");
        build_transfer_plan(d, s->L[static_cast<size_t>(l)].edges, levels[l + 1].coords, levels[l + 1].nel,
                            s->L[static_cast<size_t>(l) + 1].plan.new_of_old, s->L[static_cast<size_t>(l)].plan,
                            order_keys ? order_keys[l] : nullptr, s->L[static_cast<size_t>(l)].n_owned);
        s->L[static_cast<size_t>(l)].has_transfer = true;
    });
    lap("transfer plans");
    std::vector<LevelStaging> staging(static_cast<size_t>(nlevels));
    run_per_level(nlevels, [&](int l) {
        LevelStaging &st = staging[static_cast<size_t>(l)];
        const mgcfd_level_desc &d = levels[l];
        DeviceLevel &lv = s->L[static_cast<size_t>(l)];
        lv.info = d;
        lv.info.volumes = nullptr; lv.info.coords = nullptr; lv.info.edges = nullptr; lv.info.mg_map = nullptr;
        const int64_t nel = d.nel;
        const LevelPlan &P = lv.plan;
        const int64_t stride = int64_t(P.n_slices) * kSlice;
        std::vector<double> vol(static_cast<size_t>(stride), 1.0), cb(static_cast<size_t>(stride), 1.0);
        for (int64_t n = 0; n < nel; n++) {
            const double v = d.volumes[P.old_of_new[static_cast<size_t>(n)]];
            vol[static_cast<size_t>(n)] = v;
            cb[static_cast<size_t>(n)] = std::cbrt(v);
            if (P.old_of_new[static_cast<size_t>(n)] >= lv.n_owned) cb[static_cast<size_t>(n)] = std::numeric_limits<double>::infinity();
        }
        st.upload(lv.volumes, std::move(vol));
        st.upload(lv.cbrt_vol, std::move(cb));
        st.alloc(lv.fluxes, sizeof(double) * (static_cast<size_t>(stride) * 5));
        st.alloc(lv.residuals, sizeof(double) * (static_cast<size_t>(stride) * 5));
        st.alloc(lv.step_factors, sizeof(double) * (static_cast<size_t>(stride)));
        st.alloc(lv.sf_alt, sizeof(double) * (static_cast<size_t>(stride)));
        st.alloc(lv.min_dt, sizeof(double) * (1));
        st.upload(lv.partial_min, std::vector<double>(static_cast<size_t>((nel + 255) / 256), std::numeric_limits<double>::infinity()));
        st.alloc(lv.tile_sumsq, sizeof(double) * (static_cast<size_t>((nel + 255) / 256)));
        st.alloc(lv.sumsq, sizeof(double) * (1));
        lv.n_partials = static_cast<int>(std::min<int64_t>(1024, (nel * 5 + 255) / 256));
        st.alloc(lv.partials, sizeof(double) * (static_cast<size_t>(lv.n_partials)));
        lv.dp.nel = nel;
        lv.dp.stride = stride;
        lv.dp.n_slices = P.n_slices;
        st.upload(lv.dp.slice_row0, P.slice_row0);
        st.upload(lv.dp.rows_int, P.rows_int);
        st.upload(lv.dp.rows_bnd, P.rows_bnd);
        {
            std::vector<double> ws(P.w.size() * 4 + 2 * 4 * kSlice, 0.0);
            for (size_t e = 0; e < P.w.size(); e++) {
                const size_t row = e / kSlice, lane = e % kSlice;
                ws[(row * 4 + 0) * kSlice + lane] = P.w[e].x;
                ws[(row * 4 + 1) * kSlice + lane] = P.w[e].y;
                ws[(row * 4 + 2) * kSlice + lane] = P.w[e].z;
                ws[(row * 4 + 3) * kSlice + lane] = P.w[e].k;
            }
            st.upload(lv.dp.w, std::move(ws));
        }
        st.upload(lv.dp.old_of_new, P.old_of_new);
        lv.dp.n_tiles = P.n_tiles;
        lv.plan.nbr16.resize(P.nbr16.size() + 2 * kSlice, static_cast<uint16_t>(kT16Pad));
        st.upload(lv.dp.nbr16, P.nbr16);
        {
            std::vector<int32_t> fixed(static_cast<size_t>(P.n_tiles) * kHaloStride, -1);
            for (int32_t t = 0; t < P.n_tiles; t++)
                std::copy(P.tile_halo.begin() + P.tile_halo_ptr[static_cast<size_t>(t)],
                          P.tile_halo.begin() + P.tile_halo_ptr[static_cast<size_t>(t) + 1],
                          fixed.begin() + static_cast<size_t>(t) * kHaloStride);
            st.upload(lv.dp.tile_halo, std::move(fixed));
        }
        st.upload(lv.dp.tile_ovf_ptr, P.tile_ovf_ptr);
        st.upload(lv.dp.tile_ovf, P.tile_ovf);
        lv.row_bytes = int64_t(P.slice_row0.back()) * kSlice * 34;
        lv.dp.pad_row = P.slice_row0.back();
        lv.dp.pad_chunk = P.te_chunk_ptr.empty() ? 0 : P.te_chunk_ptr.back();
        lv.dp.n_edges = d.n_internal;
        lv.dp.n_edges_pad = (d.n_internal + 255) / 256 * 256;
        lv.plan.row_edge.resize(P.row_edge.size() + 2 * kSlice, -1);
        lv.dp.has_tail = P.has_tail ? 1 : 0;
        if (lv.dp.has_tail) {
            st.upload(lv.dp.tail.rows_main, P.rows_main);
            st.upload(lv.dp.tail.tile_ptr, P.tail_tile_ptr);
            st.upload(lv.dp.tail.rec, P.tail_rec);
            lv.plan.tail_begin.resize(static_cast<size_t>(lv.dp.stride), 0);
            lv.plan.tail_count.resize(static_cast<size_t>(lv.dp.stride), 0);
            st.upload(lv.dp.tail.begin, P.tail_begin);
            st.upload(lv.dp.tail.count, P.tail_count);
            st.alloc(lv.dp.tail.flux, sizeof(double) * static_cast<size_t>(6 * P.tail_total));
        }
        lv.dp.vin_ok = (P.halo_overflow_refs == 0 && P.halo_max <= kTile) ? 1 : 0;
        lv.dp.lds_complete = P.halo_overflow_refs == 0 ? 1 : 0;
        lv.dp.halo_max = P.halo_max;
        lv.dp.edge_once = (P.edge_once && !std::getenv("MGCFD_NO_EDGE_ONCE")) ? 1 : 0;
        if (lv.dp.edge_once) {
            lv.plan.te_slots.resize(P.te_slots.size() + 2 * kEdgeChunk, static_cast<uint16_t>(kT16Pad));
            lv.plan.te_w.resize(P.te_w.size() + 4 * kEdgeChunk, 0.0);
            lv.plan.gat16.resize(P.gat16.size() + 2 * kSlice, static_cast<uint16_t>(kT16Pad));
        }
        lv.dp.half = (P.half && !std::getenv("MGCFD_NO_HALF_ROWS")) ? 1 : 0;
        lv.dp.free_rows = (P.free_rows && !std::getenv("MGCFD_NO_HALF_ROWS")) ? 1 : 0;
        lv.dp.hr_max_rows = P.hr_max_rows;
        lv.dp.free_wide = (lv.dp.free_rows && P.free_wide) ? 1 : 0;
        if (!lv.dp.free_wide) { lv.plan.free_halo.clear(); lv.plan.free_halo.shrink_to_fit(); }
        if (lv.dp.free_rows) {
            lv.dp.hr_pad_row = P.hr_row0.back();
            lv.plan.hr_code.resize(P.hr_code.size() + 2 * kSlice, kHalfPad);
            lv.plan.hr_w.resize(P.hr_w.size() + 2 * 3 * kSlice, 0.0);
            lv.plan.hg16.resize(P.hg16.size() + 2 * kSlice, static_cast<uint16_t>(kT16Pad));
        } else {
            lv.plan.hr_code.clear(); lv.plan.hr_code.shrink_to_fit();
            lv.plan.hr_w.clear(); lv.plan.hr_w.shrink_to_fit();
            lv.plan.hg16.clear(); lv.plan.hg16.shrink_to_fit();
        }
        if (!lv.dp.edge_once) {
            lv.plan.te_slots.clear(); lv.plan.te_slots.shrink_to_fit();
            lv.plan.te_w.clear(); lv.plan.te_w.shrink_to_fit();
            lv.plan.gat16.clear(); lv.plan.gat16.shrink_to_fit();
        }
        if (lv.has_transfer) {
            st.upload(lv.dp.child_ptr, P.child_ptr);
// ... 157 lines not shown
    const int rc = guarded([&] {
        if (nlevels <= 0) throw std::invalid_argument("no levels given");
        std::vector<LevelPlan> plans(static_cast<size_t>(nlevels));
        std::vector<std::vector<mgcfd_edge>> edges(static_cast<size_t>(nlevels));
        for (int l = 0; l < nlevels; l++) {
            const mgcfd_level_desc &d = levels[l];
            if (!d.volumes || !d.edges) throw std::invalid_argument("level is missing volumes/edges");
            edges[static_cast<size_t>(l)].assign(d.edges, d.edges + d.n_edges);
            adjust_and_dampen(d, mesh_variant, edges[static_cast<size_t>(l)]);
            PlanOptions popt;
            if (const char *o = std::getenv("MGCFD_TILE_ORDER")) popt.tile_order = std::atoi(o);
            if (const char *o = std::getenv("MGCFD_TILE_CURVE")) popt.tile_curve = std::atoi(o);
            if (n_owned && n_owned[l] >= 0 && n_owned[l] < d.nel) popt.n_owned = n_owned[l];
            build_level_plan(d, edges[static_cast<size_t>(l)], popt, plans[static_cast<size_t>(l)]);
        }
        for (int l = 0; l + 1 < nlevels; l++) {
            if (!levels[l].mg_map) throw std::invalid_argument("multigrid map missing between levels");
            build_transfer_plan(levels[l], edges[static_cast<size_t>(l)], levels[l + 1].coords, levels[l + 1].nel,
                                plans[static_cast<size_t>(l) + 1].new_of_old, plans[static_cast<size_t>(l)],
                                order_keys ? order_keys[l] : nullptr, (n_owned && n_owned[l] >= 0) ? n_owned[l] : -1);
        }
        for (int l = 0; l < nlevels; l++) {
            const std::string r = audit_level_plan(levels[l], plans[static_cast<size_t>(l)], l + 1 < nlevels ? levels[l + 1].nel : -1);
            if (!r.empty()) rep += "level " + std::to_string(l) + ":\n" + r;
            if (std::getenv("MGCFD_PLAN_DIGEST")) {
                char buf[64];
                std::snprintf(buf, sizeof(buf), "digest level %d: %016llx\n", l, (unsigned long long)plan_digest(plans[static_cast<size_t>(l)]));
                rep += buf;
            }
        }
    });
    if (rc != MGCFD_OK) return rc;
    if (report && report_cap > 0) { std::snprintf(report, static_cast<size_t>(report_cap), "%s", rep.c_str()); }
    if (!rep.empty()) { g_last_error = "plan audit: " + rep; return MGCFD_ERR_ARG; }
    return MGCFD_OK;
}

int mgcfd_create(const mgcfd_level_desc *levels, int nlevels, int mesh_variant, int device, mgcfd_solver **out)
{
    REQUIRE(out);
    return guarded([&] { *out = build_solver(levels, nlevels, mesh_variant, device).release(); });
}
int mgcfd_create_partitioned(const mgcfd_level_desc *levels, int nlevels, int mesh_variant, int device,
                             const int64_t *n_owned, mgcfd_solver **out)
{
    REQUIRE(out); REQUIRE(n_owned);
    return guarded([&] { *out = build_solver(levels, nlevels, mesh_variant, device, n_owned).release(); });
}
int mgcfd_create_partitioned_mg(const mgcfd_level_desc *levels, int nlevels, int mesh_variant, int device,
                                const int64_t *n_owned, const int64_t *const *order_keys, mgcfd_solver **out)
{
    REQUIRE(out); REQUIRE(n_owned);
    return guarded([&] { *out = build_solver(levels, nlevels, mesh_variant, device, n_owned, order_keys).release(); });
}
int mgcfd_create_from_mesh(const mgcfd_mesh *m, int device, mgcfd_solver **out)
{
    REQUIRE(m); REQUIRE(out);
    return guarded([&] {
        std::vector<mgcfd_level_desc> d;
        for (auto &l : m->mesh.levels) d.push_back(l.desc());
        *out = build_solver(d.data(), static_cast<int>(d.size()), m->mesh.mesh_variant, device).release();
    });
}
void mgcfd_destroy(mgcfd_solver *s) { delete s; }

int mgcfd_set_option(mgcfd_solver *s, int option, int value)
{
    REQUIRE(s);
    return guarded([&] {
        switch (option) {
            case MGCFD_OPT_EXACT: s->opt_exact = value != 0; s->upload_optional_plans(); break;
            case MGCFD_OPT_TIMING:
                if (value < 0 || value > 4) throw std::invalid_argument("MGCFD_OPT_TIMING is 0 ... 4");
                s->use_device(); s->fold_events(); s->opt_timing = value == 3 ? 2 : value; s->timing_stride = value == 3 ? 1 : (value == 4 ? 32 : 8);
                if (const char *e = std::getenv("MGCFD_TIMING_STRIDE")) if (std::atoi(e) > 0 && value != 3) s->timing_stride = std::atoi(e);
                break;
            case MGCFD_OPT_INDIRECT_RW: s->opt_indirect_rw = value != 0; break;
            case MGCFD_OPT_CHECK_INVALID: s->opt_check = value != 0; break;
            case MGCFD_OPT_FLUX_VARIANT: s->opt_variant = value; s->upload_optional_plans(); break;
            case MGCFD_OPT_FUSE_UPDATE: s->opt_fuse = value != 0; break;
            case MGCFD_OPT_GRAPH: s->opt_graph = value != 0; break;
            case MGCFD_OPT_RANK_SPLIT: s->opt_rank_split = value < 0 ? 0 : (value > 2 ? 2 : value); break;
            case MGCFD_OPT_STAGE_WG4: s->opt_stage_wg4 = value != 0; break;
            default: throw std::invalid_argument("unknown option");
        }
    });
}
int mgcfd_level_has_half_rows(const mgcfd_solver *s, int level, int *yes)
{
    REQUIRE(s); REQUIRE(yes);
    if (level < 0 || level >= static_cast<int>(s->L.size())) { g_last_error = "level out of range"; return MGCFD_ERR_ARG; }
    *yes = s->L[static_cast<size_t>(level)].dp.half;
    return MGCFD_OK;
}
int mgcfd_level_has_order_free(const mgcfd_solver *s, int level, int *yes)
{
    REQUIRE(s); REQUIRE(yes);
    if (level < 0 || level >= static_cast<int>(s->L.size())) { g_last_error = "level out of range"; return MGCFD_ERR_ARG; }
    *yes = s->L[static_cast<size_t>(level)].dp.free_rows;
    return MGCFD_OK;
}
int mgcfd_level_stage_wg4(const mgcfd_solver *s, int level, int *yes)
{
    REQUIRE(s); REQUIRE(yes);
    if (level < 0 || level >= static_cast<int>(s->L.size())) { g_last_error = "level out of range"; return MGCFD_ERR_ARG; }
    *yes = s->stage_wg4_for(s->L[static_cast<size_t>(level)]) ? 1 : 0;
    return MGCFD_OK;
}
int mgcfd_level_has_edge_once(const mgcfd_solver *s, int level, int *yes)
{
    REQUIRE(s); REQUIRE(yes);
    if (level < 0 || level >= static_cast<int>(s->L.size())) { g_last_error = "level out of range"; return MGCFD_ERR_ARG; }
    *yes = s->L[static_cast<size_t>(level)].dp.edge_once;
    return MGCFD_OK;
}
int mgcfd_level_tiling(const mgcfd_solver *s, int level, int64_t out[10])
{
    REQUIRE(s); REQUIRE(out);
    if (level < 0 || level >= static_cast<int>(s->L.size())) { g_last_error = "level out of range"; return MGCFD_ERR_ARG; }
    const LevelPlan &P = s->L[static_cast<size_t>(level)].plan;
    out[0] = P.n_tiles;
    out[1] = P.halo_total;
    out[2] = P.halo_max;
    out[3] = kTileCap - kTile;
    out[4] = P.halo_overflow_refs;
    out[5] = P.n_internal_entries;
    out[6] = P.pad_entries;
    out[7] = P.ordered_by_boxes ? 1 : 0;
    out[8] = P.has_tail ? P.tail_total : 0;
    out[9] = 0;
    for (int32_t r : P.rows_main) out[9] += r;
    return MGCFD_OK;
}
int mgcfd_get_option(const mgcfd_solver *s, int option, int *value)
{
    REQUIRE(s); REQUIRE(value);
    switch (option) {
        case MGCFD_OPT_EXACT: *value = s->opt_exact; break;
        case MGCFD_OPT_TIMING: *value = s->opt_timing; break;
        case MGCFD_OPT_INDIRECT_RW: *value = s->opt_indirect_rw; break;
        case MGCFD_OPT_CHECK_INVALID: *value = s->opt_check; break;
        case MGCFD_OPT_FLUX_VARIANT: *value = s->opt_variant; break;
        case MGCFD_OPT_FUSE_UPDATE: *value = s->opt_fuse; break;
        case MGCFD_OPT_GRAPH: *value = s->opt_graph; break;
        case MGCFD_OPT_RANK_SPLIT: *value = s->opt_rank_split; break;
        case MGCFD_OPT_STAGE_WG4: *value = s->opt_stage_wg4; break;
        default: g_last_error = "unknown option"; return MGCFD_ERR_ARG;
    }
    return MGCFD_OK;
}
int mgcfd_set_stream(mgcfd_solver *s, void *hip_stream)
{
    REQUIRE(s);
    return guarded([&] {
        s->use_device();
        s->fold_events();
        HIP_CHECK(hipStreamSynchronize(s->stream));
        s->stream = hip_stream ? static_cast<hipStream_t>(hip_stream) : s->own_stream;
    });
}
int mgcfd_synchronize(mgcfd_solver *s)
{
    REQUIRE(s);
    return guarded([&] { s->use_device(); HIP_CHECK(hipStreamSynchronize(s->stream)); HIP_CHECK(hipGetLastError()); fail_on_ipc_timeouts(s); });
}
int mgcfd_num_levels(const mgcfd_solver *s) { return s ? static_cast<int>(s->L.size()) : 0; }
int64_t mgcfd_level_nel(const mgcfd_solver *s, int l)
{ return (s && l >= 0 && l < static_cast<int>(s->L.size())) ? s->L[static_cast<size_t>(l)].info.nel : -1; }
int64_t mgcfd_level_num_internal_edges(const mgcfd_solver *s, int l)
{ return (s && l >= 0 && l < static_cast<int>(s->L.size())) ? s->L[static_cast<size_t>(l)].info.n_internal : -1; }
int mgcfd_get_far_field(const mgcfd_solver *s, double *out17)
{
    REQUIRE(s); REQUIRE(out17);
    std::memcpy(out17, s->ff17, sizeof(double) * 17);
    return MGCFD_OK;
}

#define OP(body) REQUIRE(s); return guarded([&] { s->use_device(); body; HIP_CHECK(hipGetLastError()); })
int mgcfd_copy_old_variables(mgcfd_solver *s, int level) { OP(s->op_copy_old(level)); }
int mgcfd_compute_step_factor(mgcfd_solver *s, int level) { OP(s->op_step_factor(level)); }
int mgcfd_compute_flux_edge(mgcfd_solver *s, int level) { OP(s->op_flux(level, 1)); }
int mgcfd_compute_boundary_flux_edge(mgcfd_solver *s, int level) { OP(s->op_flux(level, 2)); }
int mgcfd_compute_wall_flux_edge(mgcfd_solver *s, int level) { OP(s->op_flux(level, 4)); }
int mgcfd_compute_fluxes(mgcfd_solver *s, int level) { OP(s->op_flux(level, 7)); }
int mgcfd_time_step(mgcfd_solver *s, int level, int j) { OP(s->op_time_step(level, j)); }
int mgcfd_zero_fluxes(mgcfd_solver *s, int level) { OP(s->op_zero_fluxes(level)); }
int mgcfd_indirect_rw(mgcfd_solver *s, int level) { OP(s->op_indirect_rw(level)); }
int mgcfd_residual(mgcfd_solver *s, int level) { OP(s->op_residual(level)); }
int mgcfd_restrict(mgcfd_solver *s, int fine_level) { OP(s->op_restrict(fine_level)); }
int mgcfd_prolong(mgcfd_solver *s, int fine_level) { OP(s->op_prolong(fine_level)); }
int mgcfd_step_factor_local(mgcfd_solver *s, int level)
{
    OP({
        if (s->mesh_variant == MGCFD_MESH_FVCORR) throw std::invalid_argument("fvcorr uses a local time step: nothing to reduce");
        s->op_step_factor_local(level, false, true);
        s->level(level).iters[MGCFD_LOOP_COMPUTE_STEP] += s->level(level).info.nel;
    });
}
int mgcfd_step_factor_min_devptr(mgcfd_solver *s, int level, void **devptr)
{ REQUIRE(devptr); OP(*devptr = s->level(level).min_dt); }
int mgcfd_step_factor_apply(mgcfd_solver *s, int level) { OP(s->op_step_factor_apply(level)); }
int mgcfd_residual_sumsq(mgcfd_solver *s, int level, void **devptr)
{ REQUIRE(devptr); OP({ s->op_sumsq(level); *devptr = s->level(level).sumsq; }); }

int mgcfd_calc_rms(mgcfd_solver *s, int level, double *rms)
{
    REQUIRE(s); REQUIRE(rms);
    return guarded([&] {
        s->use_device();
        DeviceLevel &lv = s->level(level);
        s->op_sumsq(level);
        double sum = 0.0;
        HIP_CHECK(hipMemcpyAsync(&sum, lv.sumsq, sizeof(double), hipMemcpyDeviceToHost, s->stream));
        HIP_CHECK(hipStreamSynchronize(s->stream));
        *rms = std::sqrt(sum / double(lv.n_owned));
    });
}
int mgcfd_invalid_state_location(const mgcfd_solver *s, int64_t *cell, int *cycle)
{
    REQUIRE(s);
    if (cell) *cell = s->invalid_cell;
    if (cycle) *cycle = s->invalid_cycle;
    return MGCFD_OK;
}
int mgcfd_check_for_invalid_variables(mgcfd_solver *s, int level, int64_t *bad_cell)
{
    REQUIRE(s);
    int code = MGCFD_OK;
    int rc = guarded([&] {
        s->use_device();
        DeviceLevel &lv = s->level(level);
        exact::launch_check_invalid(s->stream, lv.info.nel, lv.dp.stride, lv.q, lv.dp.old_of_new, s->err);
        code = s->read_error(bad_cell);
    });
    if (rc != MGCFD_OK) return rc;
    if (code != MGCFD_OK) g_last_error = "invalid variables detected";
    return code;
}

int mgcfd_pending_invalid_state(mgcfd_solver *s, int64_t *bad_cell)
{
    REQUIRE(s);
    int code = MGCFD_OK;
    int rc = guarded([&] { s->use_device(); code = s->read_error(bad_cell); });
    if (rc != MGCFD_OK) return rc;
    if (code != MGCFD_OK) g_last_error = "invalid variables detected";
    return code;
}

static void smooth_once(mgcfd_solver *s, int level)
{
    DeviceLevel &lv = s->level(level);
    if (s->opt_fuse && !(s->variant_for(lv) & 4) && !s->opt_indirect_rw && s->opt_timing != 1 && lv.fluxes_zero) {
        const bool global_dt = s->mesh_variant != MGCFD_MESH_FVCORR;
        bool apply_pending = global_dt;
        lv.residuals_stale = false;
        if (lv.min_ahead) {
            if (!global_dt) { lv.sf_par ^= 1; lv.apply_sf(); }
            lv.iters[MGCFD_LOOP_COMPUTE_STEP] += lv.info.nel;
        } else {
            apply_pending = s->op_step_factor(level, true, false);
        }
        const bool look_ahead = s->L.size() == 1 && lv.n_owned == lv.info.nel;
        double *const start = lv.q, *const b1 = lv.q_alt, *const b2 = lv.old_variables;
        int apply = apply_pending ? 1 : 0;
        if (apply_pending && lv.plan.n_tiles > 2048) {
            exact::launch_min_reduce(s->stream, lv.info.nel, lv.partial_min, lv.min_dt);
            apply = 2;
        }
        const bool sumsq = lv.want_sumsq && lv.n_owned == lv.info.nel;
        mgcfd_solver::Timed group(s, level, MGCFD_LOOP_FLUX, true, s->opt_timing == 2 ? MGCFD_RK : 1);
        s->op_fused_stage(level, 0, start, b1, apply, false, start);
        s->op_fused_stage(level, 1, b1, b2, 0, false, start);
        const bool lazy_res = s->L.size() == 1 && s->opt_lazy_residual;
        s->op_fused_stage(level, 2, b2, b1, 0, true, start, look_ahead, sumsq, nullptr, nullptr, 0, true, nullptr, 0, lazy_res);
        lv.have_sumsq = sumsq;
        lv.rot = (lv.rot + 1) % 3;
        lv.apply_rot();
        lv.min_ahead = look_ahead;
        lv.residuals_stale = lazy_res;
        return;
    }
    const bool apply_pending = s->op_step_factor(level, true);
    int apply0 = apply_pending ? 1 : 0;
    if (apply_pending && lv.plan.n_tiles > 2048) {
        exact::launch_min_reduce(s->stream, lv.info.nel, lv.partial_min, lv.min_dt);
        apply0 = 2;
    }
    for (int j = 0; j < MGCFD_RK; j++) {
        s->op_flux(level, 7);
        s->op_time_step(level, j, j == 0 ? apply0 : 0, j == MGCFD_RK - 1, !s->opt_indirect_rw);
        if (s->opt_indirect_rw && (j == 0 || !s->probe_first_stage_only)) { s->op_indirect_rw(level); s->op_zero_fluxes(level); }
    }
}

static void run_sweep(mgcfd_solver *s, int level)
{
    DeviceLevel &lv = s->level(level);
    const int64_t n = s->sweep_counter++;
    bool timed = s->opt_timing == 1 || (s->opt_timing == 2 && (n % s->timing_stride) == 0);
    if (s->opt_timing == 4) {
        const bool sampled = (lv.att_sweeps % s->timing_stride) == 0;
        const bool probe = sampled && s->opt_indirect_rw && (lv.att_sweeps_sampled % 4) == 0;
        lv.att_sweeps++;
        if (sampled) lv.att_sweeps_sampled++;
        if (probe) lv.att_calls_sampled[MGCFD_LOOP_INDIRECT_RW]++;
        const int keep_t = s->opt_timing, keep_p = s->opt_indirect_rw;
        s->opt_timing = sampled ? 1 : 0;
        if (keep_p) lv.iters[MGCFD_LOOP_INDIRECT_RW] += int64_t(probe ? MGCFD_RK - 1 : MGCFD_RK) * lv.info.n_internal;
        if (!probe) s->opt_indirect_rw = 0;
        s->probe_first_stage_only = true;
        try { smooth_once(s, level); } catch (...) { s->opt_timing = keep_t; s->opt_indirect_rw = keep_p; s->probe_first_stage_only = false; throw; }
        s->opt_timing = keep_t; s->opt_indirect_rw = keep_p; s->probe_first_stage_only = false;
        return;
    }
    const bool graphable = s->opt_graph && s->opt_fuse && !(s->variant_for(lv) & 4) && !s->opt_indirect_rw && !timed && lv.fluxes_zero && !lv.fluxes_stale;
    if (!graphable) {
        const int keep = s->opt_timing;
        if (!timed) s->opt_timing = 0;
        smooth_once(s, level);
        s->opt_timing = keep;
        return;
    }
    const uint64_t key = (uint64_t(level) << 32) | (uint64_t(lv.want_sumsq) << 28) | (uint64_t(lv.sf_par) << 27) | (uint64_t(lv.rot) << 25) | (uint64_t(lv.min_ahead) << 24) | (uint64_t(s->opt_exact) << 16) | (uint64_t(s->opt_stage_wg4) << 17) | (uint64_t(s->opt_check) << 8) | uint64_t(s->opt_variant & 0xFF);
    auto it = s->sweep_graphs.find(key);
    if (it == s->sweep_graphs.end()) {
        mgcfd_solver::SweepGraph g;
        int64_t before[MGCFD_NUM_LOOPS];
        std::memcpy(before, lv.iters, sizeof(before));
        const int keep = s->opt_timing;
        s->opt_timing = 0;
        hipGraph_t graph = nullptr;
        HIP_CHECK(hipStreamBeginCapture(s->stream, hipStreamCaptureModeRelaxed));
        try {
            smooth_once(s, level);
        } catch (...) {
            (void)hipStreamEndCapture(s->stream, &graph);
            if (graph) (void)hipGraphDestroy(graph);
            s->opt_timing = keep;
            throw;
        }
        s->opt_timing = keep;
        HIP_CHECK(hipStreamEndCapture(s->stream, &graph));
        HIP_CHECK(hipGraphInstantiate(&g.exec, graph, nullptr, nullptr, 0));
        HIP_CHECK(hipGraphDestroy(graph));
        for (int k = 0; k < MGCFD_NUM_LOOPS; k++) { g.iters[k] = lv.iters[k] - before[k]; lv.iters[k] = before[k]; }
        g.ahead_after = lv.min_ahead;
        g.rot_after = lv.rot;
        g.sf_par_after = lv.sf_par;
        g.sumsq_after = lv.have_sumsq;
        g.res_stale_after = lv.residuals_stale;
        it = s->sweep_graphs.emplace(key, g).first;
    }
    HIP_CHECK(hipGraphLaunch(it->second.exec, s->stream));
    lv.min_ahead = it->second.ahead_after;
    lv.rot = it->second.rot_after;
    lv.apply_rot();
    lv.sf_par = it->second.sf_par_after;
    lv.apply_sf();
    lv.have_sumsq = it->second.sumsq_after;
    lv.residuals_stale = it->second.res_stale_after;
    for (int k = 0; k < MGCFD_NUM_LOOPS; k++) lv.iters[k] += it->second.iters[k];
}

static int sweep_begin_impl(mgcfd_solver *s, int level, bool scalar)
{
    OP({
        DeviceLevel &lv = s->level(level);
        if (!lv.fluxes_zero) throw std::invalid_argument("sweep_begin needs zero fluxes (as after time_step)");
        lv.sweep_flux0_done = false;
        const bool global_dt = s->mesh_variant != MGCFD_MESH_FVCORR;
        if (lv.min_ahead) {
            if (!global_dt) { lv.sf_par ^= 1; lv.apply_sf(); }
            lv.iters[MGCFD_LOOP_COMPUTE_STEP] += lv.info.nel;
        } else {
            s->op_step_factor(level, true, false);
        }
        if (global_dt && scalar) exact::launch_min_reduce(s->stream, lv.info.nel, lv.partial_min, lv.min_dt);
    });
}
int mgcfd_sweep_flux0(mgcfd_solver *s, int level)
{
    OP({
        DeviceLevel &lv = s->level(level);
        if (!lv.fluxes_zero) throw std::invalid_argument("sweep_flux0 must follow sweep_begin");
        s->op_flux(level, 7);
        lv.sweep_flux0_done = true;
    });
}
static int sweep_end_impl(mgcfd_solver *s, int level, bool scalar)
{
    OP({
        DeviceLevel &lv = s->level(level);
        const bool global_dt = s->mesh_variant != MGCFD_MESH_FVCORR;
        const int apply = global_dt ? (scalar ? 2 : 1) : 0;
        const bool look_ahead = s->L.size() == 1 && lv.n_owned == lv.info.nel;
        double *const start = lv.q;
        double *const b1 = lv.q_alt;
        double *const b2 = lv.old_variables;
        if (lv.sweep_flux0_done && global_dt && lv.dp.vin_ok && !((s->variant_for(lv) & 2) && lv.dp.edge_once)) {
            s->op_fused_stage(level, 1, start, b2, apply, false, start, false, false, lv.fluxes);
            lv.iters[MGCFD_LOOP_TIME_STEP] += lv.info.nel;
            lv.fluxes_zero = true;
            lv.fluxes_stale = true;
            lv.sweep_flux0_done = false;
        } else {
            if (lv.sweep_flux0_done) {
                s->op_time_step(level, 0, apply, false, true, start, b1);
                lv.sweep_flux0_done = false;
            } else {
                s->settle_fluxes(lv);
                s->op_fused_stage(level, 0, start, b1, apply, false, start);
            }
            s->op_fused_stage(level, 1, b1, b2, 0, false, start);
        }
        s->op_fused_stage(level, 2, b2, b1, 0, true, start, look_ahead);
        lv.rot = (lv.rot + 1) % 3;
        lv.apply_rot();
        lv.min_ahead = look_ahead;
    });
}

int mgcfd_sweep_stage(mgcfd_solver *s, int level, int j, int partials)
{
    OP({
        DeviceLevel &lv = s->level(level);
        if (j != lv.stage_next) throw std::invalid_argument("mgcfd_sweep_stage: stages must run in order 0, 1, 2 after mgcfd_sweep_begin");
        const bool global_dt = s->mesh_variant != MGCFD_MESH_FVCORR;
        double *const start = lv.q;
        double *const b1 = lv.q_alt;
        double *const b2 = lv.old_variables;
        if (j == 0) {
            if (!lv.fluxes_zero) throw std::invalid_argument("mgcfd_sweep_stage needs zero fluxes (as after time_step)");
            s->settle_fluxes(lv);
            s->op_fused_stage(level, 0, start, b1, global_dt ? (partials ? 1 : 2) : 0, false, start);
            lv.stage_out = b1;
            lv.stage_next = 1;
        } else if (j == 1) {
// ... 17 lines not shown
int mgcfd_step_factor_partials_devptr(mgcfd_solver *s, int level, void **devptr, int *count)
{
    REQUIRE(devptr); REQUIRE(count);
    OP({ DeviceLevel &lv = s->level(level); *devptr = lv.partial_min; *count = static_cast<int>((lv.info.nel + 255) / 256); });
}

int mgcfd_smooth(mgcfd_solver *s, int level, int sweeps)
{
    OP({
        s->level(level);
        for (int k = 0; k < sweeps; k++) run_sweep(s, level);
    });
}

static void cycle_once(mgcfd_solver *s, bool capturing)
{
    const int n = static_cast<int>(s->L.size());
    auto sweep = [&](int l) { if (capturing) smooth_once(s, l); else run_sweep(s, l); };
    SumTask rms_task;
    bool rms_pending = false;
    auto transfer = [&](bool restriction, int fine, const SumTask *task) {
        const int keep = s->opt_timing;
        if (keep == 4) {
            DeviceLevel &book = s->L[static_cast<size_t>(restriction ? fine + 1 : fine)];
            const int loop = restriction ? MGCFD_LOOP_RESTRICT : MGCFD_LOOP_PROLONG;
            const bool sampled = (book.att_calls[loop] % s->timing_stride) == 0;
            book.att_calls[loop]++;
            if (sampled) book.att_calls_sampled[loop]++;
            s->opt_timing = sampled ? 1 : 0;
        }
        try { if (restriction) s->op_restrict(fine, task); else s->op_prolong(fine); } catch (...) { s->opt_timing = keep; throw; }
        s->opt_timing = keep;
    };
    for (int l = 0; l < n; l++) {
        if (l == 0) { s->L[0].want_sumsq = true; s->L[0].have_sumsq = false; }
        sweep(l);
        if (l == 0) {
            DeviceLevel &l0 = s->L[0];
            l0.want_sumsq = false;
            if (l0.have_sumsq && n > 1) {
                rms_task = SumTask{l0.tile_sumsq, static_cast<int>((l0.info.nel + 255) / 256), l0.sumsq, s->rms_ring, s->rms_count,
                                   mgcfd_solver::kRmsRing};
                rms_pending = true;
            } else if (l0.have_sumsq) {
                exact::launch_sum_partials_append(s->stream, static_cast<int>((l0.info.nel + 255) / 256), l0.tile_sumsq, l0.sumsq,
                                                  s->rms_ring, s->rms_count, mgcfd_solver::kRmsRing);
            } else {
                s->op_sumsq(0);
                exact::launch_append_scalar(s->stream, l0.sumsq, s->rms_ring, s->rms_count, mgcfd_solver::kRmsRing);
            }
        }
        if (l + 1 < n) { transfer(true, l, (l == 0 && rms_pending) ? &rms_task : nullptr); rms_pending = false; }
    }
    for (int l = n - 2; l >= 0; l--) {
        transfer(false, l, nullptr);
        if (l > 0) sweep(l);
    }
}

int mgcfd_run_cycles(mgcfd_solver *s, int cycles, double *rms_out)
{
    REQUIRE(s);
    int code = MGCFD_OK, failed_cycle = -1, seq_before = 0, seq_per_cycle = 0;
    int rc = guarded([&] {
        s->use_device();
        if (!s->rms_ring) {
            s->rms_ring = dev_alloc<double>(mgcfd_solver::kRmsRing);
            s->rms_count = dev_alloc<int>(1);
        }
        const size_t nl = s->L.size();
        std::vector<double> sums;
        sums.reserve(static_cast<size_t>(cycles > 0 ? cycles : 0));
        seq_before = s->check_seq;
        for (int done = 0; done < cycles;) {
            const int chunk = std::min(cycles - done, mgcfd_solver::kRmsRing);
            HIP_CHECK(hipMemsetAsync(s->rms_count, 0, sizeof(int), s->stream));
            hipEvent_t att0 = nullptr, att1 = nullptr;
            if (s->opt_timing == 4) { att0 = s->get_event(); att1 = s->get_event(); HIP_CHECK(hipEventRecord(att0, s->stream)); }
            bool graphable = s->opt_graph && s->opt_fuse && !s->opt_indirect_rw && s->opt_timing == 0;
            for (auto &lv : s->L) graphable = graphable && lv.fluxes_zero && !lv.fluxes_stale && !(s->variant_for(lv) & 4);
            graphable = graphable && nl <= 8;
            if (graphable) {
                for (int c = 0; c < chunk; c++) {
                    uint64_t key = (uint64_t(s->opt_exact) << 16) | (uint64_t(s->opt_stage_wg4) << 17) | (uint64_t(s->opt_check) << 8) | uint64_t(s->opt_variant & 0xFF);
                    for (size_t l = 0; l < nl && l < 8; l++) key |= (uint64_t(s->L[l].min_ahead) << (24 + l)) | (uint64_t(s->L[l].rot) << (32 + 2 * l)) | (uint64_t(s->L[l].sf_par) << (48 + l));
                    auto it = s->cycle_graphs.find(key);
                    if (it == s->cycle_graphs.end()) {
                        mgcfd_solver::CycleGraph g;
                        std::vector<std::vector<int64_t>> before(nl);
                        std::vector<bool> ahead_before, stale_before;
                        std::vector<int> rot_before, sf_before;
                        for (size_t l = 0; l < nl; l++) {
                            before[l].assign(s->L[l].iters, s->L[l].iters + MGCFD_NUM_LOOPS);
                            ahead_before.push_back(s->L[l].min_ahead);
                            stale_before.push_back(s->L[l].residuals_stale);
                            rot_before.push_back(s->L[l].rot);
                            sf_before.push_back(s->L[l].sf_par);
                        }
                        hipGraph_t graph = nullptr;
                        HIP_CHECK(hipStreamBeginCapture(s->stream, hipStreamCaptureModeRelaxed));
                        try {
                            cycle_once(s, true);
                        } catch (...) {
                            (void)hipStreamEndCapture(s->stream, &graph);
                            if (graph) (void)hipGraphDestroy(graph);
                            throw;
                        }
                        HIP_CHECK(hipStreamEndCapture(s->stream, &graph));
                        HIP_CHECK(hipGraphInstantiate(&g.exec, graph, nullptr, nullptr, 0));
                        HIP_CHECK(hipGraphDestroy(graph));
                        g.iters.resize(nl);
                        for (size_t l = 0; l < nl; l++) {
                            for (int k = 0; k < MGCFD_NUM_LOOPS; k++) {
                                g.iters[l].push_back(s->L[l].iters[k] - before[l][static_cast<size_t>(k)]);
                                s->L[l].iters[k] = before[l][static_cast<size_t>(k)];
                            }
                            g.ahead_after.push_back(s->L[l].min_ahead);
                            g.rot_after.push_back(s->L[l].rot);
                            g.sf_par_after.push_back(s->L[l].sf_par);
                            g.res_stale_after.push_back(s->L[l].residuals_stale);
                            s->L[l].residuals_stale = stale_before[l];
                            s->L[l].min_ahead = ahead_before[l];
                            s->L[l].rot = rot_before[l];
                            s->L[l].apply_rot();
                            s->L[l].sf_par = sf_before[l];
                            s->L[l].apply_sf();
                        }
                        it = s->cycle_graphs.emplace(key, std::move(g)).first;
                    }
                    HIP_CHECK(hipGraphLaunch(it->second.exec, s->stream));
                    for (size_t l = 0; l < nl; l++) {
                        for (int k = 0; k < MGCFD_NUM_LOOPS; k++) s->L[l].iters[k] += it->second.iters[l][static_cast<size_t>(k)];
                        s->L[l].min_ahead = it->second.ahead_after[l];
                        s->L[l].residuals_stale = it->second.res_stale_after[l];
                        s->L[l].rot = it->second.rot_after[l];
                        s->L[l].apply_rot();
                        s->L[l].sf_par = it->second.sf_par_after[l];
                        s->L[l].apply_sf();
                    }
                }
            } else {
                for (int c = 0; c < chunk; c++) {
                    cycle_once(s, false);
                    if (c == 0) seq_per_cycle = s->check_seq - seq_before;
                }
            }
            if (att1) HIP_CHECK(hipEventRecord(att1, s->stream));
            const size_t at = sums.size();
            sums.resize(at + static_cast<size_t>(chunk));
            HIP_CHECK(hipMemcpyAsync(sums.data() + at, s->rms_ring, sizeof(double) * chunk, hipMemcpyDeviceToHost, s->stream));
            int seq = 0;
            code = s->read_error(nullptr, &seq);
            if (att1) {
                float ms = 0.f;
                HIP_CHECK(hipEventElapsedTime(&ms, att0, att1));
                s->att_total += double(ms) * 1e-3;
                s->free_events.push_back(att0); s->free_events.push_back(att1);
            }
            if (code != MGCFD_OK) {
                if (seq_per_cycle > 0 && seq > seq_before)
                    failed_cycle = done + std::min(chunk - 1, (seq - 1 - seq_before) / seq_per_cycle);
                done += chunk;
                break;
            }
            done += chunk;
            seq_before = 0;
        }
        if (rms_out) {
            const double nan = std::numeric_limits<double>::quiet_NaN();
            for (int c = 0; c < cycles; c++)
                rms_out[c] = (c < static_cast<int>(sums.size()) && (failed_cycle < 0 || c < failed_cycle))
                                 ? std::sqrt(sums[static_cast<size_t>(c)] / double(s->L[0].n_owned)) : nan;
        }
        HIP_CHECK(hipGetLastError());
    });
    if (rc != MGCFD_OK) return rc;
    if (code != MGCFD_OK) {
        s->invalid_cycle = failed_cycle;
        g_last_error = std::string("check_for_invalid_variables: ") +
                       (code == MGCFD_ERR_NAN ? "NaN/Inf" : code == MGCFD_ERR_NEG_DENSITY ? "negative density" : "negative density*energy") +
                       " at cell " + std::to_string(s->invalid_cell) +
                       (failed_cycle >= 0 ? " in cycle " + std::to_string(failed_cycle + 1) : std::string(" during the cycles"));
    }
    return code;
}

static double *array_ptr(DeviceLevel &lv, int which, int *ncols)
{
    *ncols = 5;
    switch (which) {
        case MGCFD_ARR_VARIABLES: return lv.q;
        case MGCFD_ARR_OLD_VARIABLES: return lv.old_variables;
        case MGCFD_ARR_FLUXES: return lv.fluxes;
        case MGCFD_ARR_RESIDUALS: return lv.residuals;
        case MGCFD_ARR_STEP_FACTORS: *ncols = 1; return lv.step_factors;
        case MGCFD_ARR_VOLUMES: *ncols = 1; return lv.volumes;
        case MGCFD_ARR_STAGE:
            if (!lv.stage_out) throw std::invalid_argument("MGCFD_ARR_STAGE: no mgcfd_sweep_stage has run on this level");
            return lv.stage_out;
        default: throw std::invalid_argument("unknown array id");
    }
}
int mgcfd_get_array(mgcfd_solver *s, int level, int which, double *out)
{
    REQUIRE(s); REQUIRE(out);
    return guarded([&] {
        s->use_device();
        DeviceLevel &lv = s->level(level);
        int nc = 0;
        double *src = (s->settle_residuals(lv), array_ptr(lv, which, &nc));
        if (which == MGCFD_ARR_FLUXES) s->settle_fluxes(lv);
        const int64_t stride = lv.dp.stride;
        std::vector<double> tmp(static_cast<size_t>(stride) * nc);
        HIP_CHECK(hipMemcpyAsync(tmp.data(), src, tmp.size() * sizeof(double), hipMemcpyDeviceToHost, s->stream));
        HIP_CHECK(hipStreamSynchronize(s->stream));
        fail_on_ipc_timeouts(s);
// ... 1731 lines not shown
```

mg-cfd-app-plain_amd/mgcfd/api.py:

```python
from __future__ import annotations

import ctypes as C
import os
import sys
from typing import List, Optional, Sequence

import numpy as np

from .meshgen import EDGE_DTYPE, LevelMesh, MultigridMesh, to_edge_arrays

PKG_DIR = os.path.dirname(os.path.abspath(__file__))
CSRC_DIR = os.path.normpath(os.path.join(PKG_DIR, "..", "csrc"))
LIB_PATH = os.environ.get("MGCFD_LIB") or os.path.join(CSRC_DIR, "libmgcfd_hip.so")

NVAR = 5
RK = 3
LOOPS = ("flux", "update", "compute_step", "time_step", "restrict", "prolong", "indirect_rw")
ARR = {"variables": 0, "old_variables": 1, "fluxes": 2, "residuals": 3, "step_factors": 4, "volumes": 5, "stage": 6}
OPT = {"exact": 0, "timing": 1, "indirect_rw": 2, "check_invalid": 3, "flux_variant": 4, "fuse_update": 5, "graph": 6, "rank_split": 7, "stage_wg4": 8}
ERR_NAMES = {0: "OK", 1: "ERR_ARG", 2: "ERR_IO", 3: "ERR_HIP", 4: "ERR_NAN", 5: "ERR_NEG_DENSITY",
             6: "ERR_NEG_ENERGY", 7: "ERR_VALIDATION"}

_vp = C.c_void_p
_i64 = C.c_int64


class LevelDesc(C.Structure):
    _fields_ = [("nel", _i64), ("n_edges", _i64), ("n_internal", _i64), ("n_boundary", _i64),
                ("n_wall", _i64), ("internal_start", _i64), ("boundary_start", _i64), ("wall_start", _i64),
                ("volumes", _vp), ("coords", _vp), ("edges", _vp), ("mg_map", _vp), ("mgc", _i64)]


class MgcfdError(RuntimeError):
    def __init__(self, code: int, message: str):
        super().__init__(f"{ERR_NAMES.get(code, code)}: {message}")
        self.code = code


_SIGNATURES = [
    ("mgcfd_last_error", C.c_char_p, []),
    ("mgcfd_abi_version", C.c_int, []),
    ("mgcfd_mesh_load", C.c_int, [C.c_char_p, C.c_char_p, C.c_int, C.POINTER(_vp)]),
    ("mgcfd_mesh_load_ex", C.c_int, [C.c_char_p, C.c_char_p, C.c_int, C.c_int, C.POINTER(_vp)]),
    ("mgcfd_mesh_free", None, [_vp]),
    ("mgcfd_mesh_num_levels", C.c_int, [_vp]),
    ("mgcfd_mesh_variant", C.c_int, [_vp]),
    ("mgcfd_mesh_size", C.c_int, [_vp]),
    ("mgcfd_mesh_level", C.c_int, [_vp, C.c_int, C.POINTER(LevelDesc)]),
    ("mgcfd_write_array", C.c_int, [C.c_char_p, _vp, _i64, C.c_int]),
    ("mgcfd_identify_differences", C.c_int, [_vp, _vp, _i64, C.c_int, C.POINTER(_i64)]),
    ("mgcfd_create", C.c_int, [C.POINTER(LevelDesc), C.c_int, C.c_int, C.c_int, C.POINTER(_vp)]),
    ("mgcfd_plan_audit", C.c_int, [C.POINTER(LevelDesc), C.c_int, C.c_int, C.POINTER(_i64), C.POINTER(C.POINTER(_i64)), C.c_char_p, _i64]),
    ("mgcfd_create_partitioned_mg", C.c_int, [C.POINTER(LevelDesc), C.c_int, C.c_int, C.c_int, C.POINTER(_i64),
                                                 C.POINTER(C.POINTER(_i64)), C.POINTER(_vp)]),
    ("mgcfd_create_from_mesh", C.c_int, [_vp, C.c_int, C.POINTER(_vp)]),
    ("mgcfd_create_partitioned", C.c_int, [C.POINTER(LevelDesc), C.c_int, C.c_int, C.c_int, C.POINTER(_i64), C.POINTER(_vp)]),
    ("mgcfd_halo_plan", C.c_int, [_vp, C.c_int, _i64, _vp, C.POINTER(C.c_int)]),
    ("mgcfd_halo_pack", C.c_int, [_vp, C.c_int, C.c_int, C.c_int, _vp]),
    ("mgcfd_halo_unpack", C.c_int, [_vp, C.c_int, C.c_int, C.c_int, _vp]),
    ("mgcfd_destroy", None, [_vp]),
    ("mgcfd_set_option", C.c_int, [_vp, C.c_int, C.c_int]),
    ("mgcfd_level_has_edge_once", C.c_int, [_vp, C.c_int, C.POINTER(C.c_int)]),
    ("mgcfd_level_has_half_rows", C.c_int, [_vp, C.c_int, C.POINTER(C.c_int)]),
    ("mgcfd_pending_invalid_state", C.c_int, [_vp, C.POINTER(C.c_int64)]),
    ("mgcfd_level_has_order_free", C.c_int, [_vp, C.c_int, C.POINTER(C.c_int)]),
    ("mgcfd_level_stage_wg4", C.c_int, [_vp, C.c_int, C.POINTER(C.c_int)]),
    ("mgcfd_level_tiling", C.c_int, [_vp, C.c_int, C.POINTER(C.c_int64)]),
    ("mgcfd_invalid_state_location", C.c_int, [_vp, C.POINTER(C.c_int64), C.POINTER(C.c_int)]),
    ("mgcfd_get_option", C.c_int, [_vp, C.c_int, C.POINTER(C.c_int)]),
    ("mgcfd_set_stream", C.c_int, [_vp, _vp]),
    ("mgcfd_synchronize", C.c_int, [_vp]),
    ("mgcfd_num_levels", C.c_int, [_vp]),
    ("mgcfd_level_nel", _i64, [_vp, C.c_int]),
    ("mgcfd_level_num_internal_edges", _i64, [_vp, C.c_int]),
    ("mgcfd_get_far_field", C.c_int, [_vp, _vp]),
    ("mgcfd_copy_old_variables", C.c_int, [_vp, C.c_int]),
    ("mgcfd_compute_step_factor", C.c_int, [_vp, C.c_int]),
    ("mgcfd_compute_flux_edge", C.c_int, [_vp, C.c_int]),
    ("mgcfd_compute_boundary_flux_edge", C.c_int, [_vp, C.c_int]),
    ("mgcfd_compute_wall_flux_edge", C.c_int, [_vp, C.c_int]),
    ("mgcfd_compute_fluxes", C.c_int, [_vp, C.c_int]),
    ("mgcfd_time_step", C.c_int, [_vp, C.c_int, C.c_int]),
    ("mgcfd_zero_fluxes", C.c_int, [_vp, C.c_int]),
    ("mgcfd_indirect_rw", C.c_int, [_vp, C.c_int]),
    ("mgcfd_residual", C.c_int, [_vp, C.c_int]),
    ("mgcfd_calc_rms", C.c_int, [_vp, C.c_int, C.POINTER(C.c_double)]),
    ("mgcfd_check_for_invalid_variables", C.c_int, [_vp, C.c_int, C.POINTER(_i64)]),
    ("mgcfd_restrict", C.c_int, [_vp, C.c_int]),
    ("mgcfd_prolong", C.c_int, [_vp, C.c_int]),
    ("mgcfd_smooth", C.c_int, [_vp, C.c_int, C.c_int]),
    ("mgcfd_run_cycles", C.c_int, [_vp, C.c_int, _vp]),
    ("mgcfd_get_array", C.c_int, [_vp, C.c_int, C.c_int, _vp]),
    ("mgcfd_set_array", C.c_int, [_vp, C.c_int, C.c_int, _vp]),
    ("mgcfd_array_devptr", C.c_int, [_vp, C.c_int, C.c_int, C.POINTER(_vp), C.POINTER(C.c_int64)]),
    ("mgcfd_array_written", C.c_int, [_vp, C.c_int, C.c_int]),
    ("mgcfd_get_edges", C.c_int, [_vp, C.c_int, _vp]),
    ("mgcfd_accept_restricted", C.c_int, [_vp, C.c_int, _vp]),
    ("mgcfd_get_loop_iters", C.c_int, [_vp, C.c_int, _vp]),
    ("mgcfd_get_loop_times", C.c_int, [_vp, C.c_int, _vp]),
    ("mgcfd_reset_monitoring", C.c_int, [_vp]),
    ("mgcfd_get_flux_kernel_time", C.c_int, [_vp, C.c_int, C.POINTER(C.c_double), C.POINTER(_i64)]),
    ("mgcfd_bench_flux", C.c_int, [_vp, C.c_int, C.c_int, C.POINTER(C.c_double)]),
    ("mgcfd_bench_indirect_rw", C.c_int, [_vp, C.c_int, C.c_int, C.POINTER(C.c_double)]),
    ("mgcfd_bench_stream_ceiling", C.c_int, [_vp, C.c_int, C.c_int, C.POINTER(C.c_double)]),
    ("mgcfd_device_warm_up", C.c_int, [C.c_int]),
    ("mgcfd_step_factor_local", C.c_int, [_vp, C.c_int]),
    ("mgcfd_step_factor_min_devptr", C.c_int, [_vp, C.c_int, C.POINTER(_vp)]),
    ("mgcfd_step_factor_partials_devptr", C.c_int, [_vp, C.c_int, C.POINTER(_vp), C.POINTER(C.c_int)]),
    ("mgcfd_sweep_stage", C.c_int, [_vp, C.c_int, C.c_int, C.c_int]),
    ("mgcfd_sweep_begin_partials", C.c_int, [_vp, C.c_int]),
    ("mgcfd_sweep_end_partials", C.c_int, [_vp, C.c_int]),
    ("mgcfd_step_factor_apply", C.c_int, [_vp, C.c_int]),
    ("mgcfd_sweep_begin", C.c_int, [_vp, C.c_int]),
    ("mgcfd_sweep_flux0", C.c_int, [_vp, C.c_int]),
    ("mgcfd_sweep_end", C.c_int, [_vp, C.c_int]),
    ("mgcfd_residual_sumsq", C.c_int, [_vp, C.c_int, C.POINTER(_vp)]),
    ("mgcfd_rccl_unique_id", C.c_int, [_vp]),
    ("mgcfd_rank_attach_rccl", C.c_int, [_vp, C.c_int, C.c_int, _vp]),
    ("mgcfd_rank_detach", C.c_int, [_vp]),
    ("mgcfd_rank_set_halo", C.c_int, [_vp, C.c_int, C.c_int, C.POINTER(C.c_int), C.POINTER(_i64), C.POINTER(_vp), C.POINTER(_i64), C.POINTER(_vp)]),
    ("mgcfd_rank_halo_info", C.c_int, [_vp, C.c_int, C.POINTER(_i64)]),
    ("mgcfd_rank_exchange", C.c_int, [_vp, C.c_int]),
    ("mgcfd_rank_sweeps", C.c_int, [_vp, C.c_int, C.c_int]),
    ("mgcfd_rank_residual_sumsq", C.c_int, [_vp, C.c_int, C.POINTER(C.c_double)]),
    ("mgcfd_group_create", C.c_int, [C.c_int, C.POINTER(_vp), C.POINTER(_vp)]),
    ("mgcfd_group_destroy", None, [_vp]),
    ("mgcfd_group_exchange", C.c_int, [_vp, C.c_int]),
    ("mgcfd_rank_attach_plain", C.c_int, [_vp, C.c_int, C.c_int]),
    ("mgcfd_rank_ipc_export_size", C.c_int, [_vp, C.c_int, C.POINTER(C.c_int64)]),
    ("mgcfd_rank_ipc_export", C.c_int, [_vp, C.c_int, _vp]),
    ("mgcfd_rank_ipc_attach", C.c_int, [_vp, C.c_int, C.c_int, C.POINTER(_vp)]),
    ("mgcfd_rank_ipc_status", C.c_int, [_vp, C.c_int, C.POINTER(C.c_int)]),
    ("mgcfd_rank_info", C.c_int, [_vp, C.POINTER(C.c_int)]),
    ("mgcfd_rank_graph_status", C.c_int, [_vp, C.c_int, C.POINTER(_i64)]),
    ("mgcfd_group_cycles", C.c_int, [_vp, C.c_int, C.POINTER(C.c_double)]),
    ("mgcfd_rank_cycles", C.c_int, [_vp, C.c_int, C.POINTER(C.c_double)]),
    ("mgcfd_rank_ipc_detach", C.c_int, [_vp, C.c_int]),
    ("mgcfd_group_sweeps", C.c_int, [_vp, C.c_int, C.c_int]),
    ("mgcfd_group_sweeps_rms", C.c_int, [_vp, C.c_int, C.c_int, C.POINTER(C.c_double)]),
    ("mgcfd_group_rms", C.c_int, [_vp, C.c_int, C.POINTER(C.c_double)]),
    ("mgcfd_group_synchronize", C.c_int, [_vp]),
]
EXPORTED_SYMBOLS = tuple(name for name, _, _ in _SIGNATURES)

_lib: Optional[C.CDLL] = None


def load_library(path: Optional[str] = None) -> C.CDLL:
    global _lib
# ... 128 lines not shown
    def from_mesh(cls, mesh: Mesh, device: int = 0) -> "Solver":
        lib = load_library()
        h = _vp()
        _check(lib, lib.mgcfd_create_from_mesh(mesh.handle, device, C.byref(h)))
        return cls(h, lib)

    @classmethod
    def from_arrays(cls, levels: Sequence[dict], mesh_variant: int, device: int = 0, n_owned=None, order_keys=None) -> "Solver":
        lib = load_library()
        descs, keep = _level_descs(levels)
        h = _vp()
        if n_owned is None:
            _check(lib, lib.mgcfd_create(descs, len(levels), mesh_variant, device, C.byref(h)))
        elif order_keys is None:
            owned = (_i64 * len(levels))(*[int(v) for v in n_owned])
            _check(lib, lib.mgcfd_create_partitioned(descs, len(levels), mesh_variant, device, owned, C.byref(h)))
        else:
            owned = (_i64 * len(levels))(*[int(v) for v in n_owned])
            keys = [None if k is None else np.ascontiguousarray(k, dtype=np.int64) for k in order_keys]
            keep += keys
            kp = (C.POINTER(_i64) * len(levels))(*[C.cast(_ptr(k), C.POINTER(_i64)) if k is not None else C.POINTER(_i64)() for k in keys])
            _check(lib, lib.mgcfd_create_partitioned_mg(descs, len(levels), mesh_variant, device, owned, kp, C.byref(h)))
        return cls(h, lib)

    @classmethod
    def from_generated(cls, mg: MultigridMesh, device: int = 0) -> "Solver":
        return cls.from_arrays(generated_to_levels(mg), mg.mesh_variant, device)

    def _c(self, rc):
        _check(self.lib, rc)

    def close(self):
        if getattr(self, "handle", None):
            self.lib.mgcfd_destroy(self.handle)
            self.handle = None

    def __del__(self):
        try:
            self.close()
        except Exception:
            pass

    def set_option(self, name: str, value: int):
        self._c(self.lib.mgcfd_set_option(self.handle, OPT[name], int(value)))

    def array_devptr(self, l: int, name: str):
        p, n = _vp(), C.c_int64()
        self._c(self.lib.mgcfd_array_devptr(self.handle, l, ARR[name], C.byref(p), C.byref(n)))
        return p.value, n.value

    def accept_restricted(self, fine: int, dev_ptr: int):
        self._c(self.lib.mgcfd_accept_restricted(self.handle, fine, C.c_void_p(dev_ptr)))

    def array_written(self, l: int, name: str):
        self._c(self.lib.mgcfd_array_written(self.handle, l, ARR[name]))

    def invalid_state_location(self):
        cell, cycle = C.c_int64(-1), C.c_int(-1)
        self._c(self.lib.mgcfd_invalid_state_location(self.handle, C.byref(cell), C.byref(cycle)))
        return cell.value, cycle.value

    def tiling(self, l: int) -> dict:
        out = (C.c_int64 * 10)()
        self._c(self.lib.mgcfd_level_tiling(self.handle, l, out))
        keys = ("tiles", "halo_nodes", "halo_max", "halo_capacity", "overflow_refs", "row_entries", "padding_entries", "coordinate_boxes",
                "list_entries", "loop_rows")
        return dict(zip(keys, (int(v) for v in out)))

    def has_half_rows(self, l: int) -> bool:
        yes = C.c_int(0)
        self._c(self.lib.mgcfd_level_has_half_rows(self.handle, l, C.byref(yes)))
        return bool(yes.value)

    def has_order_free(self, l: int) -> bool:
        yes = C.c_int(0)
        self._c(self.lib.mgcfd_level_has_order_free(self.handle, l, C.byref(yes)))
        return bool(yes.value)

    def stage_wg4(self, l: int) -> bool:
        yes = C.c_int(0)
        self._c(self.lib.mgcfd_level_stage_wg4(self.handle, l, C.byref(yes)))
        return bool(yes.value)

    def has_edge_once(self, l: int) -> bool:
        v = C.c_int()
        self._c(self.lib.mgcfd_level_has_edge_once(self.handle, l, C.byref(v)))
        return bool(v.value)

    def get_option(self, name: str) -> int:
        v = C.c_int()
        self._c(self.lib.mgcfd_get_option(self.handle, OPT[name], C.byref(v)))
        return v.value

    def set_stream(self, stream_handle: Optional[int]):
        if stream_handle is not None and int(stream_handle) == 0:
            raise ValueError("stream handle 0 is the legacy default stream; make a torch.cuda.Stream() current "
                             "(torch.cuda.set_stream) and pass its .cuda_stream, or pass None for the solver's own stream")
        self._c(self.lib.mgcfd_set_stream(self.handle, _vp(stream_handle) if stream_handle is not None else None))
        self._stream_handle = int(stream_handle) if stream_handle is not None else None

    def synchronize(self):
        self._c(self.lib.mgcfd_synchronize(self.handle))

    @property
    def num_levels(self) -> int:
        return self.lib.mgcfd_num_levels(self.handle)

    def nel(self, l: int) -> int:
        return self.lib.mgcfd_level_nel(self.handle, l)

    def num_internal_edges(self, l: int) -> int:
        return self.lib.mgcfd_level_num_internal_edges(self.handle, l)

    def far_field(self) -> np.ndarray:
        out = np.zeros(17)
        self._c(self.lib.mgcfd_get_far_field(self.handle, _ptr(out)))
        return out

    def copy_old_variables(self, l): self._c(self.lib.mgcfd_copy_old_variables(self.handle, l))
    def compute_step_factor(self, l): self._c(self.lib.mgcfd_compute_step_factor(self.handle, l))
    def compute_flux_edge(self, l): self._c(self.lib.mgcfd_compute_flux_edge(self.handle, l))
    def compute_boundary_flux_edge(self, l): self._c(self.lib.mgcfd_compute_boundary_flux_edge(self.handle, l))
    def compute_wall_flux_edge(self, l): self._c(self.lib.mgcfd_compute_wall_flux_edge(self.handle, l))
    def compute_fluxes(self, l): self._c(self.lib.mgcfd_compute_fluxes(self.handle, l))
    def time_step(self, l, j): self._c(self.lib.mgcfd_time_step(self.handle, l, j))
    def zero_fluxes(self, l): self._c(self.lib.mgcfd_zero_fluxes(self.handle, l))
    def indirect_rw(self, l): self._c(self.lib.mgcfd_indirect_rw(self.handle, l))
    def residual(self, l): self._c(self.lib.mgcfd_residual(self.handle, l))
    def restrict(self, fine): self._c(self.lib.mgcfd_restrict(self.handle, fine))
    def prolong(self, fine): self._c(self.lib.mgcfd_prolong(self.handle, fine))

    def calc_rms(self, l) -> float:
        v = C.c_double()
        self._c(self.lib.mgcfd_calc_rms(self.handle, l, C.byref(v)))
        return v.value

    def check_for_invalid_variables(self, l):
        bad = _i64(-1)
        rc = self.lib.mgcfd_check_for_invalid_variables(self.handle, l, C.byref(bad))
        return rc, bad.value

    def pending_invalid_state(self):
        bad = _i64(-1)
        rc = self.lib.mgcfd_pending_invalid_state(self.handle, C.byref(bad))
        return rc, bad.value

    def smooth(self, l: int, sweeps: int = 1):
        self._c(self.lib.mgcfd_smooth(self.handle, l, sweeps))

    def run_cycles(self, cycles: int) -> np.ndarray:
        rms = np.zeros(max(cycles, 1))
        self._c(self.lib.mgcfd_run_cycles(self.handle, cycles, _ptr(rms)))
        return rms[:cycles]

    def get(self, l: int, name: str) -> np.ndarray:
        ncols = 1 if name in ("step_factors", "volumes") else NVAR
        out = np.zeros(self.nel(l) * ncols)
        self._c(self.lib.mgcfd_get_array(self.handle, l, ARR[name], _ptr(out)))
        return out.reshape(-1, ncols) if ncols > 1 else out

    def set(self, l: int, name: str, values: np.ndarray):
        a = np.ascontiguousarray(values, dtype=np.float64).ravel()
        ncols = 1 if name in ("step_factors", "volumes") else NVAR
        assert a.size == self.nel(l) * ncols
        self._c(self.lib.mgcfd_set_array(self.handle, l, ARR[name], _ptr(a)))

# ... 193 lines not shown
```

Baseline: 51960 Medges/s.

## Fold look-ahead step-factor minimum into atomic min cells instead of partial-min scan

Replaces the per-block scan of partial minima at the start of the first RK stage with eight order-preserving uint64 keys, updated by atomic min in the look-ahead stage and read directly by every block. Two banks ping-pong between sweeps, and the unused bank is reset in-kernel by block 0. It also preloads cbrt_vol earlier in the ROLE 3 path. This removes the kPartPre partial-min loads and the LDS reduction per block, at the cost of global atomics and extra state tracking in the graph cache keys.

```diff
diff --git a/include/mgcfd.h b/include/mgcfd.h
--- a/include/mgcfd.h
+++ b/include/mgcfd.h
@@ -40,7 +40,8 @@
     MGCFD_OPT_FUSE_UPDATE = 5,
     MGCFD_OPT_GRAPH = 6,
     MGCFD_OPT_RANK_SPLIT = 7,
-    MGCFD_OPT_STAGE_WG4 = 8
+    MGCFD_OPT_STAGE_WG4 = 8,
+    MGCFD_OPT_MIN_CELLS = 9
 };
 
 typedef struct { int64_t a, b; double x, y, z; } mgcfd_edge;
@@ -92,6 +93,7 @@
 int mgcfd_level_has_half_rows(const mgcfd_solver *s, int level, int *yes);
 int mgcfd_level_has_order_free(const mgcfd_solver *s, int level, int *yes);
 int mgcfd_level_stage_wg4(const mgcfd_solver *s, int level, int *yes);
+int mgcfd_level_min_cells(const mgcfd_solver *s, int level, int *yes);
 int mgcfd_level_tiling(const mgcfd_solver *s, int level, int64_t out[10]);
 int mgcfd_get_option(const mgcfd_solver *s, int option, int *value);
 int mgcfd_set_stream(mgcfd_solver *s, void *hip_stream);
diff --git a/mg-cfd-app-plain_amd/csrc/device_plan.hpp b/mg-cfd-app-plain_amd/csrc/device_plan.hpp
--- a/mg-cfd-app-plain_amd/csrc/device_plan.hpp
+++ b/mg-cfd-app-plain_amd/csrc/device_plan.hpp
@@ -3,6 +3,7 @@
 #include <hip/hip_runtime.h>
 #include <cstdint>
 
+#include "min_key.hpp"
 #include "preprocess.hpp"
 
 namespace mgcfd {
@@ -69,6 +70,9 @@
     double *next_partial_min = nullptr;
     const double *cbrt_vol = nullptr;
     double *next_legacy_sf = nullptr;
+    unsigned long long *next_min_cells = nullptr;
+    const unsigned long long *min_cells = nullptr;
+    unsigned long long *min_cells_reset = nullptr;
     const int32_t *tile_list = nullptr;
     int32_t n_list = 0;
     int64_t nel_active = 0;
diff --git a/mg-cfd-app-plain_amd/csrc/kernels.hip b/mg-cfd-app-plain_amd/csrc/kernels.hip
--- a/mg-cfd-app-plain_amd/csrc/kernels.hip
+++ b/mg-cfd-app-plain_amd/csrc/kernels.hip
@@ -538,6 +538,8 @@
     constexpr int kPartPre = 6;
     double *const s_pm = lds.s_pm;
     double pmv[kPartPre];
+    const bool cells = FUSE && ROLE == 0 && fs.min_cells != nullptr;
+    unsigned long long ckey[kMinCells];
 
     const int tid = threadIdx.x;
     const int lane = tid & 63;
@@ -619,7 +621,7 @@
             if (!SLIM) e1 = load_row<LOADK>(nbr16, w, n_int > 1 ? row0 + 1 : pad_row, lane);
         }
     }
-    if (FUSE && ROLE == 0) {
+    if (FUSE && ROLE == 0 && !cells) {
 #pragma unroll
         for (int u = 0; u < kPartPre; u++) {
             const int k = threadIdx.x + u * kBlock;
@@ -639,7 +641,7 @@
         a3 = fluxes[3 * stride + i]; a4 = fluxes[4 * stride + i];
     }
     const int32_t ovf0 = tile_ovf_ptr[t];
-    if (FUSE && ROLE == 0) {
+    if (FUSE && ROLE == 0 && !cells) {
         double pm = pmv[0];
 #pragma unroll
         for (int u = 1; u < kPartPre; u++) pm = fmin(pm, pmv[u]);
@@ -650,6 +652,11 @@
     PH_MARK(0);
     __syncthreads();
     PH_MARK(1);
+    if (cells) {
+#pragma unroll
+        for (int c = 0; c < kMinCells; c++) ckey[c] = fs.min_cells[c * kMinCellStride];
+    }
+    if (FUSE && ROLE == 0 && fs.min_cells_reset && block == 0 && tid < kMinCells) fs.min_cells_reset[tid * kMinCellStride] = kMinKeyEmpty;
 
 #define MGCFD_ROW_PAIR()                                                                                     \
     do {                                                                                                     \
@@ -688,6 +695,7 @@
         if (e_first < tl_e) { tl_r0 = tp.rec[3 * int64_t(e_first)]; tl_r1 = tp.rec[3 * int64_t(e_first) + 1]; tl_r2 = tp.rec[3 * int64_t(e_first) + 2]; }
     }
     double r0 = 0.0, r1 = 0.0, r2 = 0.0, r3 = 0.0, r4 = 0.0, sfv = 0.0;
+    double cbv = 0.0;
 #define MGCFD_ROW_ONE()                                                                                      \
     do {                                                                                                     \
             const uint32_t s0 = e0.code & kT16SlotMask;                                                      \
@@ -716,6 +724,7 @@
                 r3 = fs.old_variables[3 * stride + i]; r4 = fs.old_variables[4 * stride + i];
             }
             sfv = (ROLE == 0 ? fs.volumes : fs.step_factors)[i];
+            if (ROLE == 3) cbv = fs.cbrt_vol[i];
         }
         if (r < n_int) MGCFD_ROW_ONE();
     } else
@@ -744,6 +753,7 @@
                 r3 = fs.old_variables[3 * stride + i]; r4 = fs.old_variables[4 * stride + i];
             }
             sfv = ((ROLE == 0 || ROLE == 5) ? fs.volumes : fs.step_factors)[i];
+            if (ROLE == 3 && !TAIL) cbv = fs.cbrt_vol[i];
         }
         if (r < n_int) MGCFD_ROW_PAIR();
     }
@@ -850,8 +860,15 @@
     if (i < nel) {
         double sf = sfv;
         if (ROLE == 0 || ROLE == 5) {
-            min_dt = s_pm[0];
-            for (int wv = 1; wv < kBlock / 64; wv++) min_dt = fmin(min_dt, s_pm[wv]);
+            if (cells) {
+                unsigned long long k = ckey[0];
+#pragma unroll
+                for (int c = 1; c < kMinCells; c++) k = ckey[c] < k ? ckey[c] : k;
+                min_dt = min_key_value(k);
+            } else {
+                min_dt = s_pm[0];
+                for (int wv = 1; wv < kBlock / 64; wv++) min_dt = fmin(min_dt, s_pm[wv]);
+            }
             sf = min_dt / sfv;
             fs.step_factors[i] = sf;
         }
@@ -877,7 +894,7 @@
         }
         if (ROLE == 3) {
             const Derived d = derive(rho, mx, my, mz, en);
-            const double dt = fs.cbrt_vol[i] / (d.speed + d.c);
+            const double dt = (TAIL ? fs.cbrt_vol[i] : cbv) / (d.speed + d.c);
             sf_next = 0.5 * dt;
         } else if (ROLE == 4) {
             const Derived d = derive(rho, mx, my, mz, en);
@@ -920,6 +937,9 @@
             double m = s_next[0][0], sum = s_next[1][0];
             for (int wv = 1; wv < kBlock / 64; wv++) { m = fmin(m, s_next[0][wv]); sum += s_next[1][wv]; }
             if (ROLE == 3) fs.next_partial_min[t] = m;
+            if (ROLE == 3 && fs.next_min_cells)
+                __hip_atomic_fetch_min(fs.next_min_cells + (block & unsigned(kMinCells - 1)) * kMinCellStride, min_key(m), __ATOMIC_RELAXED,
+                                       __HIP_MEMORY_SCOPE_AGENT);
             if (fs.sumsq_partial) fs.sumsq_partial[t] = sum;
         }
     }
@@ -2240,6 +2260,8 @@
     const int64_t nel_arg = (fused && fs.nel_active > 0) ? fs.nel_active : p.nel;
     const dim3 grid(part ? fs.n_list : p.n_tiles);
     if (part && fs.n_list <= 0) return;
+    const bool cells = fused && (fs.min_cells || fs.min_cells_reset || fs.next_min_cells);
+    auto no_cells = [&] { if (cells) throw std::logic_error("step-factor cells passed to a stage kernel other than k_flux_tile"); };
 
 #define MGCFD_TILE_LAUNCH_T(WMODE, FUSE, ACC, ROLE, TAIL)                                                      \
     hipLaunchKernelGGL((k_flux_tile<((TAIL) && ((ACC) || (ROLE) == 5)) ? 2 : 3, WMODE, FUSE, ACC, ROLE, TAIL>), grid, block, 0, st, q, p.tile_halo,     \
@@ -2302,6 +2324,7 @@
     }
 #ifdef MGCFD_ORDER_FREE
     if ((variant & 64) && p.free_rows && (classes & 1) && !(fused && fs.vin_flux) && !part && !(fused && fs.nel_active > 0)) {
+        no_cells();
 #define MGCFD_FREE_LAUNCH_L(FUSE, ACC, CAP, LONG)                                                               \
     hipLaunchKernelGGL((k_flux_free<FUSE, ACC, CAP, LONG>), grid, block, 0, st, q, p.tile_halo, uint32_t(p.n_tiles), \
                        p.hr_pad_row, p.stride, p.nel, p.hr_row0, p.hr_code, p.hr_w, p.slice_row0,               \
@@ -2341,6 +2364,7 @@
     }
 #endif
     if ((variant & 32) && p.half && (classes & 1) && !(fused && fs.vin_flux) && !part) {
+        no_cells();
 #define MGCFD_HALF_LAUNCH(FUSE, ACC)                                                                            \
     hipLaunchKernelGGL((k_flux_half<FUSE, ACC>), grid, block, 0, st, q, p.tile_halo, uint32_t(p.n_tiles),       \
                        p.hr_pad_row, p.stride, p.nel, p.hr_row0, p.hr_code, p.hr_w, p.hg16, p.slice_row0,       \
@@ -2353,6 +2377,7 @@
     }
     const bool loadk = (variant & 1) == 0;
     if ((variant & 2) && p.edge_once && (classes & 1) && !part) {
+        no_cells();
 #define MGCFD_EO_LAUNCH(LOADK, FUSE, ACC)                                                                      \
     hipLaunchKernelGGL((k_flux_edge_once<LOADK, FUSE, ACC>), grid, block, 0, st, q, p.tile_halo,               \
                        uint32_t(p.n_tiles), p.pad_row, p.stride, p.nel, p.te_chunk_ptr, p.te_count,            \
diff --git a/mg-cfd-app-plain_amd/csrc/min_key.hpp b/mg-cfd-app-plain_amd/csrc/min_key.hpp
--- /dev/null
+++ b/mg-cfd-app-plain_amd/csrc/min_key.hpp
@@ -0,0 +1,35 @@
+#pragma once
+
+#include <cstdint>
+#include <cstring>
+
+#if defined(__HIPCC__)
+#define MGCFD_HD __host__ __device__
+#else
+#define MGCFD_HD
+#endif
+
+namespace mgcfd {
+
+constexpr int kMinCells = 8;
+constexpr int kMinCellStride = 32;
+
+constexpr unsigned long long kMinKeyEmpty = ~0ull;
+
+MGCFD_HD inline unsigned long long min_key(double x)
+{
+    if (x != x) return kMinKeyEmpty;
+    unsigned long long b;
+    std::memcpy(&b, &x, sizeof(b));
+    return (b >> 63) ? ~b : (b | 0x8000000000000000ull);
+}
+
+MGCFD_HD inline double min_key_value(unsigned long long k)
+{
+    const unsigned long long b = (k >> 63) ? (k & 0x7FFFFFFFFFFFFFFFull) : ~k;
+    double x;
+    std::memcpy(&x, &b, sizeof(x));
+    return x;
+}
+
+}
diff --git a/mg-cfd-app-plain_amd/csrc/solver.cpp b/mg-cfd-app-plain_amd/csrc/solver.cpp
--- a/mg-cfd-app-plain_amd/csrc/solver.cpp
+++ b/mg-cfd-app-plain_amd/csrc/solver.cpp
@@ -123,6 +123,13 @@
     int64_t total_recv() const { return recv_off.empty() ? 0 : recv_off.back(); }
 };
 
+struct AheadFlag {
+    bool on = false;
+    bool cells = false;
+    AheadFlag &operator=(bool v) { on = v; cells = false; return *this; }
+    operator bool() const { return on; }
+};
+
 struct DeviceLevel {
     mgcfd_level_desc info{};
     std::vector<mgcfd_edge> edges;
@@ -137,7 +144,9 @@
     bool want_sumsq = false;
     bool have_sumsq = false;
     int64_t row_bytes = 0;
-    bool min_ahead = false;
+    AheadFlag min_ahead;
+    unsigned long long *min_cells = nullptr;
+    int cells_bank = 1;
     double *sf_alt = nullptr;
     int sf_par = 0;
     double *sfb[2] = {nullptr, nullptr};
@@ -183,6 +192,7 @@
     double ff17[17] = {0};
     unsigned long long *err = nullptr;
     int opt_exact = 1, opt_timing = 0, opt_indirect_rw = 0, opt_check = 1, opt_variant = -1, opt_fuse = 1, opt_graph = 0, opt_stage_wg4 = 1;
+    int opt_min_cells = 1;
     int opt_rank_split = 1;
     bool opt_lazy_residual = !(std::getenv("MGCFD_LAZY_RESIDUAL") && std::atoi(std::getenv("MGCFD_LAZY_RESIDUAL")) == 0);
     int check_seq = 0;
@@ -194,9 +204,9 @@
     bool probe_first_stage_only = false;
     int64_t sweep_counter = 0;
     bool in_timed_group = false;
-    struct SweepGraph { hipGraphExec_t exec = nullptr; int64_t iters[MGCFD_NUM_LOOPS] = {0}; bool ahead_after = false; int rot_after = 0; int sf_par_after = 0; bool sumsq_after = false, res_stale_after = false; };
+    struct SweepGraph { hipGraphExec_t exec = nullptr; int64_t iters[MGCFD_NUM_LOOPS] = {0}; AheadFlag ahead_after; int cells_bank_after = 1; int rot_after = 0; int sf_par_after = 0; bool sumsq_after = false, res_stale_after = false; };
     std::map<uint64_t, SweepGraph> sweep_graphs;
-    struct CycleGraph { hipGraphExec_t exec = nullptr; std::vector<std::vector<int64_t>> iters; std::vector<bool> ahead_after, res_stale_after; std::vector<int> rot_after, sf_par_after; };
+    struct CycleGraph { hipGraphExec_t exec = nullptr; std::vector<std::vector<int64_t>> iters; std::vector<AheadFlag> ahead_after; std::vector<bool> res_stale_after; std::vector<int> rot_after, sf_par_after, cells_bank_after; };
     std::map<uint64_t, CycleGraph> cycle_graphs;
     static constexpr int kRmsRing = 4096;
     double *rms_ring = nullptr;
@@ -363,6 +373,12 @@
         }
         return lv.dp.n_tiles > 3 * n_cus;
     }
+    bool min_cells_for(const DeviceLevel &lv) const
+    {
+        if (!opt_exact || !opt_min_cells || mesh_variant == MGCFD_MESH_FVCORR) return false;
+        const int v = variant_for(lv, true);
+        return !(v & 4) && !((v & 2) && lv.dp.edge_once) && !((v & 32) && lv.dp.half);
+    }
     void op_flux(int l, int classes)
     {
         DeviceLevel &lv = level(l);
@@ -382,10 +398,14 @@
                         const double *old = nullptr, bool look_ahead = false, bool sumsq = false,
                         const double *vin_flux = nullptr, const int32_t *tile_list = nullptr, int32_t n_list = 0,
                         bool count_iters = true, const double *min_list = nullptr, int n_min = 0, bool lazy_residual = false,
-                        const StagePush *push = nullptr)
+                        const StagePush *push = nullptr, const unsigned long long *cells_in = nullptr,
+                        unsigned long long *cells_reset = nullptr, unsigned long long *cells_out = nullptr)
     {
         DeviceLevel &lv = level(l);
-        const FusedStep fs = fused_step(l, j, out, apply_min, with_residual, old, look_ahead, sumsq, vin_flux, tile_list, n_list, min_list, n_min, lazy_residual);
+        FusedStep fs = fused_step(l, j, out, apply_min, with_residual, old, look_ahead, sumsq, vin_flux, tile_list, n_list, min_list, n_min, lazy_residual);
+        fs.min_cells = cells_in;
+        fs.min_cells_reset = cells_reset;
+        fs.next_min_cells = cells_out;
         Timed t(this, l, MGCFD_LOOP_FLUX, true);
         if (opt_exact) exact::launch_flux(stream, lv.dp, in, ff, lv.fluxes, 7, 0, variant_for(lv, true) | (stage_wg4_for(lv) ? kVariantStageWg4 : 0), &fs, push);
         else fast::launch_flux(stream, lv.dp, in, ff, lv.fluxes, 7, 0, variant_for(lv, true), &fs, push);
@@ -732,6 +752,7 @@
         st.alloc(lv.sf_alt, sizeof(double) * (static_cast<size_t>(stride)));
         st.alloc(lv.min_dt, sizeof(double) * (1));
         st.upload(lv.partial_min, std::vector<double>(static_cast<size_t>((nel + 255) / 256), std::numeric_limits<double>::infinity()));
+        st.upload(lv.min_cells, std::vector<unsigned long long>(2 * kMinCells * kMinCellStride, kMinKeyEmpty));
         st.alloc(lv.tile_sumsq, sizeof(double) * (static_cast<size_t>((nel + 255) / 256)));
         st.alloc(lv.sumsq, sizeof(double) * (1));
         lv.n_partials = static_cast<int>(std::min<int64_t>(1024, (nel * 5 + 255) / 256));
@@ -1055,6 +1076,7 @@
             case MGCFD_OPT_GRAPH: s->opt_graph = value != 0; break;
             case MGCFD_OPT_RANK_SPLIT: s->opt_rank_split = value < 0 ? 0 : (value > 2 ? 2 : value); break;
             case MGCFD_OPT_STAGE_WG4: s->opt_stage_wg4 = value != 0; break;
+            case MGCFD_OPT_MIN_CELLS: s->opt_min_cells = value != 0; break;
             default: throw std::invalid_argument("unknown option");
         }
     });
@@ -1078,6 +1100,14 @@
     REQUIRE(s); REQUIRE(yes);
     if (level < 0 || level >= static_cast<int>(s->L.size())) { g_last_error = "level out of range"; return MGCFD_ERR_ARG; }
     *yes = s->stage_wg4_for(s->L[static_cast<size_t>(level)]) ? 1 : 0;
+    return MGCFD_OK;
+}
+int mgcfd_level_min_cells(const mgcfd_solver *s, int level, int *yes)
+{
+    REQUIRE(s); REQUIRE(yes);
+    if (level < 0 || level >= static_cast<int>(s->L.size())) { g_last_error = "level out of range"; return MGCFD_ERR_ARG; }
+    const DeviceLevel &lv = s->L[static_cast<size_t>(level)];
+    *yes = (lv.min_ahead && lv.min_ahead.cells && s->min_cells_for(lv)) ? 1 : 0;
     return MGCFD_OK;
 }
 int mgcfd_level_has_edge_once(const mgcfd_solver *s, int level, int *yes)
@@ -1118,6 +1148,7 @@
         case MGCFD_OPT_GRAPH: *value = s->opt_graph; break;
         case MGCFD_OPT_RANK_SPLIT: *value = s->opt_rank_split; break;
         case MGCFD_OPT_STAGE_WG4: *value = s->opt_stage_wg4; break;
+        case MGCFD_OPT_MIN_CELLS: *value = s->opt_min_cells; break;
         default: g_last_error = "unknown option"; return MGCFD_ERR_ARG;
     }
     return MGCFD_OK;
@@ -1242,15 +1273,25 @@
             apply = 2;
         }
         const bool sumsq = lv.want_sumsq && lv.n_owned == lv.info.nel;
+        const bool cells = s->min_cells_for(lv);
+        const bool cells_fold = cells && look_ahead;
+        const unsigned long long *cells_in = (cells && apply == 1 && lv.min_ahead.cells) ? lv.min_cells + lv.cells_bank * kMinCells * kMinCellStride : nullptr;
+        unsigned long long *const cells_next = lv.min_cells + (lv.cells_bank ^ 1) * kMinCells * kMinCellStride;
         mgcfd_solver::Timed group(s, level, MGCFD_LOOP_FLUX, true, s->opt_timing == 2 ? MGCFD_RK : 1);
-        s->op_fused_stage(level, 0, start, b1, apply, false, start);
+        s->op_fused_stage(level, 0, start, b1, apply, false, start, false, false, nullptr, nullptr, 0, true, nullptr, 0, false, nullptr,
+                          cells_in, cells_fold ? cells_next : nullptr);
         s->op_fused_stage(level, 1, b1, b2, 0, false, start);
         const bool lazy_res = s->L.size() == 1 && s->opt_lazy_residual;
-        s->op_fused_stage(level, 2, b2, b1, 0, true, start, look_ahead, sumsq, nullptr, nullptr, 0, true, nullptr, 0, lazy_res);
+        s->op_fused_stage(level, 2, b2, b1, 0, true, start, look_ahead, sumsq, nullptr, nullptr, 0, true, nullptr, 0, lazy_res, nullptr,
+                          nullptr, nullptr, cells_fold ? cells_next : nullptr);
         lv.have_sumsq = sumsq;
         lv.rot = (lv.rot + 1) % 3;
         lv.apply_rot();
         lv.min_ahead = look_ahead;
+        if (cells_fold) {
+            lv.cells_bank ^= 1;
+            lv.min_ahead.cells = true;
+        }
         lv.residuals_stale = lazy_res;
         return;
     }
@@ -1295,7 +1336,7 @@
         s->opt_timing = keep;
         return;
     }
-    const uint64_t key = (uint64_t(level) << 32) | (uint64_t(lv.want_sumsq) << 28) | (uint64_t(lv.sf_par) << 27) | (uint64_t(lv.rot) << 25) | (uint64_t(lv.min_ahead) << 24) | (uint64_t(s->opt_exact) << 16) | (uint64_t(s->opt_stage_wg4) << 17) | (uint64_t(s->opt_check) << 8) | uint64_t(s->opt_variant & 0xFF);
+    const uint64_t key = (uint64_t(level) << 32) | (uint64_t(lv.want_sumsq) << 28) | (uint64_t(lv.sf_par) << 27) | (uint64_t(lv.rot) << 25) | (uint64_t(lv.min_ahead) << 24) | (uint64_t(s->opt_exact) << 16) | (uint64_t(s->opt_stage_wg4) << 17) | (uint64_t(s->opt_min_cells) << 18) | (uint64_t(lv.min_ahead.cells) << 19) | (uint64_t(lv.cells_bank) << 20) | (uint64_t(s->opt_check) << 8) | uint64_t(s->opt_variant & 0xFF);
     auto it = s->sweep_graphs.find(key);
     if (it == s->sweep_graphs.end()) {
         mgcfd_solver::SweepGraph g;
@@ -1319,6 +1360,7 @@
         HIP_CHECK(hipGraphDestroy(graph));
         for (int k = 0; k < MGCFD_NUM_LOOPS; k++) { g.iters[k] = lv.iters[k] - before[k]; lv.iters[k] = before[k]; }
         g.ahead_after = lv.min_ahead;
+        g.cells_bank_after = lv.cells_bank;
         g.rot_after = lv.rot;
         g.sf_par_after = lv.sf_par;
         g.sumsq_after = lv.have_sumsq;
@@ -1327,6 +1369,7 @@
     }
     HIP_CHECK(hipGraphLaunch(it->second.exec, s->stream));
     lv.min_ahead = it->second.ahead_after;
+    lv.cells_bank = it->second.cells_bank_after;
     lv.rot = it->second.rot_after;
     lv.apply_rot();
     lv.sf_par = it->second.sf_par_after;
@@ -1510,17 +1553,20 @@
             graphable = graphable && nl <= 8;
             if (graphable) {
                 for (int c = 0; c < chunk; c++) {
-                    uint64_t key = (uint64_t(s->opt_exact) << 16) | (uint64_t(s->opt_stage_wg4) << 17) | (uint64_t(s->opt_check) << 8) | uint64_t(s->opt_variant & 0xFF);
+                    uint64_t key = (uint64_t(s->opt_exact) << 16) | (uint64_t(s->opt_stage_wg4) << 17) | (uint64_t(s->opt_min_cells) << 18) | (uint64_t(s->opt_check) << 8) | uint64_t(s->opt_variant & 0xFF);
                     for (size_t l = 0; l < nl && l < 8; l++) key |= (uint64_t(s->L[l].min_ahead) << (24 + l)) | (uint64_t(s->L[l].rot) << (32 + 2 * l)) | (uint64_t(s->L[l].sf_par) << (48 + l));
+                    key |= (uint64_t(s->L[0].min_ahead.cells) << 19) | (uint64_t(s->L[0].cells_bank) << 20);
                     auto it = s->cycle_graphs.find(key);
                     if (it == s->cycle_graphs.end()) {
                         mgcfd_solver::CycleGraph g;
                         std::vector<std::vector<int64_t>> before(nl);
-                        std::vector<bool> ahead_before, stale_before;
-                        std::vector<int> rot_before, sf_before;
+                        std::vector<AheadFlag> ahead_before;
+                        std::vector<bool> stale_before;
+                        std::vector<int> rot_before, sf_before, bank_before;
                         for (size_t l = 0; l < nl; l++) {
                             before[l].assign(s->L[l].iters, s->L[l].iters + MGCFD_NUM_LOOPS);
                             ahead_before.push_back(s->L[l].min_ahead);
+                            bank_before.push_back(s->L[l].cells_bank);
                             stale_before.push_back(s->L[l].residuals_stale);
                             rot_before.push_back(s->L[l].rot);
                             sf_before.push_back(s->L[l].sf_par);
@@ -1544,6 +1590,8 @@
                                 s->L[l].iters[k] = before[l][static_cast<size_t>(k)];
                             }
                             g.ahead_after.push_back(s->L[l].min_ahead);
+                            g.cells_bank_after.push_back(s->L[l].cells_bank);
+                            s->L[l].cells_bank = bank_before[l];
                             g.rot_after.push_back(s->L[l].rot);
                             g.sf_par_after.push_back(s->L[l].sf_par);
                             g.res_stale_after.push_back(s->L[l].residuals_stale);
@@ -1560,6 +1608,7 @@
                     for (size_t l = 0; l < nl; l++) {
                         for (int k = 0; k < MGCFD_NUM_LOOPS; k++) s->L[l].iters[k] += it->second.iters[l][static_cast<size_t>(k)];
                         s->L[l].min_ahead = it->second.ahead_after[l];
+                        s->L[l].cells_bank = it->second.cells_bank_after[l];
                         s->L[l].residuals_stale = it->second.res_stale_after[l];
                         s->L[l].rot = it->second.rot_after[l];
                         s->L[l].apply_rot();
diff --git a/mg-cfd-app-plain_amd/mgcfd/api.py b/mg-cfd-app-plain_amd/mgcfd/api.py
--- a/mg-cfd-app-plain_amd/mgcfd/api.py
+++ b/mg-cfd-app-plain_amd/mgcfd/api.py
@@ -17,7 +17,7 @@
 RK = 3
 LOOPS = ("flux", "update", "compute_step", "time_step", "restrict", "prolong", "indirect_rw")
 ARR = {"variables": 0, "old_variables": 1, "fluxes": 2, "residuals": 3, "step_factors": 4, "volumes": 5, "stage": 6}
-OPT = {"exact": 0, "timing": 1, "indirect_rw": 2, "check_invalid": 3, "flux_variant": 4, "fuse_update": 5, "graph": 6, "rank_split": 7, "stage_wg4": 8}
+OPT = {"exact": 0, "timing": 1, "indirect_rw": 2, "check_invalid": 3, "flux_variant": 4, "fuse_update": 5, "graph": 6, "rank_split": 7, "stage_wg4": 8, "min_cells": 9}
 ERR_NAMES = {0: "OK", 1: "ERR_ARG", 2: "ERR_IO", 3: "ERR_HIP", 4: "ERR_NAN", 5: "ERR_NEG_DENSITY",
              6: "ERR_NEG_ENERGY", 7: "ERR_VALIDATION"}
 
@@ -65,6 +65,7 @@
     ("mgcfd_pending_invalid_state", C.c_int, [_vp, C.POINTER(C.c_int64)]),
     ("mgcfd_level_has_order_free", C.c_int, [_vp, C.c_int, C.POINTER(C.c_int)]),
     ("mgcfd_level_stage_wg4", C.c_int, [_vp, C.c_int, C.POINTER(C.c_int)]),
+    ("mgcfd_level_min_cells", C.c_int, [_vp, C.c_int, C.POINTER(C.c_int)]),
     ("mgcfd_level_tiling", C.c_int, [_vp, C.c_int, C.POINTER(C.c_int64)]),
     ("mgcfd_invalid_state_location", C.c_int, [_vp, C.POINTER(C.c_int64), C.POINTER(C.c_int)]),
     ("mgcfd_get_option", C.c_int, [_vp, C.c_int, C.POINTER(C.c_int)]),
@@ -359,6 +360,11 @@
         self._c(self.lib.mgcfd_level_stage_wg4(self.handle, l, C.byref(yes)))
         return bool(yes.value)
 
+    def min_cells(self, l: int) -> bool:
+        yes = C.c_int(0)
+        self._c(self.lib.mgcfd_level_min_cells(self.handle, l, C.byref(yes)))
+        return bool(yes.value)
+
     def has_edge_once(self, l: int) -> bool:
         v = C.c_int()
         self._c(self.lib.mgcfd_level_has_edge_once(self.handle, l, C.byref(v)))
```

New measurement: 52140 Medges/s, median of 5. No clear change (+0.3%).
